# raadyn/aztotmd

Measured on AMD Instinct MI355X. Metric: ns_per_day, higher is better.
Workload: dtype f64; 1 GPU; 1 000 188 Ar, LJ rc 8.5 A, FCC 63^3 a=5.735 jitter 0.15, dt 1 fs, NVE, init_vel zero (BASELINE config '1 000 000 Ar LJ', SURVEY C4); n_atoms=1000188, n_cells=68921, decomposition=single GPU, transport=single GPU, rccl_ranks=0, pair_variant=0, sort_interval=105, sort_violations=0, pair_lists=1, cells_without_list=0, kernel_timing=off

## Files before the change

aztotmd_amd/api.py:

```python
import ctypes as C
import enum
import os
import subprocess

import numpy as np

_HERE = os.path.dirname(os.path.abspath(__file__))
_LIB = None

STAT_FIELDS = ("step", "time", "engTot", "engKin", "engVdW", "engCoul", "engElecField", "engTemp", "engPot", "temperature",
               "posMom", "negMom", "posCross", "negCross", "pressure", "pairs_dropped", "n_cells", "nose_chit", "nose_conint",
               "engBond", "engAngle", "engCoulRec", "engCoulConst", "sort_interval", "sort_violations", "pair_lists", "cells_without_list", "rebuilds", "skin")


class AztotError(RuntimeError):
    def __init__(self, code, msg):
        super().__init__("aztot error %d: %s" % (code, msg))
        self.code = code


class _Species(C.Structure):
    _fields_ = [("name", C.c_char * 8), ("mass_amu", C.c_double), ("charge", C.c_double), ("frozen", C.c_int32),
                ("radA", C.c_double), ("radB", C.c_double), ("mxEng", C.c_double)]


class _Vdw(C.Structure):
    _fields_ = [("spec_a", C.c_int32), ("spec_b", C.c_int32), ("type", C.c_int32), ("rcut", C.c_double), ("p", C.c_double * 5)]


class _Control(C.Structure):
    _fields_ = [("timestep", C.c_double), ("nstep", C.c_int32), ("nequil", C.c_int32), ("eqfreq", C.c_int32),
                ("temperature", C.c_double), ("tstat_type", C.c_int32), ("tstat_tau", C.c_double), ("elec_type", C.c_int32),
                ("r_real", C.c_double), ("alpha", C.c_double), ("init_vel", C.c_int32), ("init_vel_par", C.c_double * 3),
                ("elecfield", C.c_double * 3), ("use_cell_list", C.c_int32), ("cell_list", C.c_double), ("stat", C.c_int32),
                ("ewald_k", C.c_int32 * 3)]


_dp = C.POINTER(C.c_double)
_ip = C.POINTER(C.c_int32)


class _System(C.Structure):
    _fields_ = [("n_atoms", C.c_int32), ("n_species", C.c_int32), ("n_vdw", C.c_int32), ("box", C.c_double * 3),
                ("types", _ip), ("x", _dp), ("y", _dp), ("z", _dp), ("vx", _dp), ("vy", _dp), ("vz", _dp),
                ("species", C.POINTER(_Species)), ("vdw", C.POINTER(_Vdw)), ("control", _Control)]


class _BondType(C.Structure):
    _fields_ = [("spec_a", C.c_int32), ("spec_b", C.c_int32), ("type", C.c_int32), ("p", C.c_double * 5)]


class _AngleType(C.Structure):
    _fields_ = [("central", C.c_int32), ("type", C.c_int32), ("k", C.c_double), ("cos0", C.c_double)]


class _Bonded(C.Structure):
    _fields_ = [("n_bond_types", C.c_int32), ("n_angle_types", C.c_int32), ("n_bonds", C.c_int32), ("n_angles", C.c_int32),
                ("bond_types", C.POINTER(_BondType)), ("angle_types", C.POINTER(_AngleType)),
                ("bond_a", _ip), ("bond_b", _ip), ("bond_type", _ip),
                ("angle_c", _ip), ("angle_l1", _ip), ("angle_l2", _ip), ("angle_type", _ip)]


class _Options(C.Structure):
    _fields_ = [("struct_size", C.c_uint32), ("device", C.c_int32), ("initial_forces", C.c_int32), ("center_box", C.c_int32), ("seed", C.c_uint64),
                ("pair_variant", C.c_int32), ("cell_size", C.c_double), ("use_graph", C.c_int32), ("profile", C.c_int32),
                ("sort_every", C.c_int32), ("skin", C.c_double), ("waves_per_cell", C.c_int32), ("energies_every_step", C.c_int32),
                ("loopback_ranks", C.c_int32), ("reserved", C.c_int32 * 5)]


class _Stats(C.Structure):
    _fields_ = [("step", C.c_int64), ("time", C.c_double), ("engTot", C.c_double), ("engKin", C.c_double), ("engVdW", C.c_double),
                ("engCoul", C.c_double), ("engElecField", C.c_double), ("engTemp", C.c_double), ("engPot", C.c_double),
                ("temperature", C.c_double), ("posMom", C.c_double * 3), ("negMom", C.c_double * 3), ("posCross", C.c_int64 * 3),
                ("negCross", C.c_int64 * 3), ("pressure", C.c_double), ("pairs_dropped", C.c_int64), ("n_cells", C.c_int64),
                ("nose_chit", C.c_double), ("nose_conint", C.c_double), ("engBond", C.c_double), ("engAngle", C.c_double),
                ("engCoulRec", C.c_double), ("engCoulConst", C.c_double), ("sort_interval", C.c_int64), ("sort_violations", C.c_int64),
                ("pair_lists", C.c_int64), ("cells_without_list", C.c_int64), ("rebuilds", C.c_int64), ("skin", C.c_double)]


class _CnColumn(C.Structure):
    _fields_ = [("central", C.c_int32), ("ligand", C.c_int32), ("radius", C.c_double)]


class _AdfColumn(C.Structure):
    _fields_ = [("central", C.c_int32), ("ligand_a", C.c_int32), ("ligand_b", C.c_int32), ("reserved", C.c_int32), ("radius_a", C.c_double), ("radius_b", C.c_double)]


class _BooParams(C.Structure):
    _fields_ = [("radius", C.c_double), ("central_mask", C.c_int32), ("ligand_mask", C.c_int32), ("n_orders", C.c_int32), ("orders", C.c_int32 * 4),
                ("n_bins", C.c_int32), ("reserved", C.c_int32)]


class _Stress(C.Structure):
    _fields_ = [("step", C.c_int64), ("time", C.c_double), ("volume", C.c_double), ("kinetic", C.c_double * 6), ("virial", C.c_double * 6),
                ("pressure", C.c_double * 6), ("pressure_iso", C.c_double), ("eng_vdw", C.c_double), ("eng_coul", C.c_double),
                ("pairs", C.c_int64), ("pairs_dropped", C.c_int64)]


class _Clock(C.Structure):
    _fields_ = [("step", C.c_int64), ("nose_chit", C.c_double), ("nose_conint", C.c_double), ("eng_kin", C.c_double)]


class _State(C.Structure):
    _fields_ = [("n_atoms", C.c_int32)] + [(k, _dp) for k in ("x", "y", "z", "vx", "vy", "vz", "fx", "fy", "fz", "U", "radius")] + [("types", _ip)]


SENDRECV_FN = C.CFUNCTYPE(C.c_int, C.c_void_p, C.c_int, C.c_void_p, C.c_int64, C.c_int, C.c_void_p, C.c_int64, C.POINTER(C.c_int64))
ALLREDUCE_FN = C.CFUNCTYPE(C.c_int, C.c_void_p, _dp, C.c_int)

EXPORTS = ("aztot_device_count", "aztot_device_synchronize", "aztot_init_md", "aztot_model_create", "aztot_model_set_bonded", "aztot_model_query", "aztot_model_species_name", "aztot_model_nucleus_name", "aztot_free_md", "aztot_default_options",
           "aztot_init_device", "aztot_free_device", "aztot_step", "aztot_sync", "aztot_forces", "aztot_get_stats", "aztot_species_crossings", "aztot_md_to_host",
           "aztot_set_state", "aztot_get_clock", "aztot_set_clock", "aztot_cell_table", "aztot_kernel_times", "aztot_reset_kernel_times", "aztot_set_profile", "aztot_comm_id_bytes", "aztot_comm_make_id", "aztot_comm_selftest", "aztot_comm_ranks",
           "aztot_init_device_slab", "aztot_rdf_setup", "aztot_rdf_sample", "aztot_rdf_reset", "aztot_rdf_shape", "aztot_rdf_counts", "aztot_rdf_values",
           "aztot_cn_setup", "aztot_cn_sample", "aztot_cn_shape", "aztot_cn_per_atom", "aztot_cn_table",
           "aztot_tcf_setup", "aztot_tcf_sample", "aztot_tcf_reset", "aztot_tcf_shape", "aztot_tcf_sums", "aztot_tcf_values",
           "aztot_stress_setup", "aztot_stress_sample", "aztot_stress_get", "aztot_stress_per_atom",
           "aztot_adf_setup", "aztot_adf_sample", "aztot_adf_reset", "aztot_adf_shape", "aztot_adf_edges", "aztot_adf_counts", "aztot_adf_values",
           "aztot_adf_neighbours",
           "aztot_sk_setup", "aztot_sk_sample", "aztot_sk_reset", "aztot_sk_shape", "aztot_sk_vectors", "aztot_sk_amplitudes", "aztot_sk_sums", "aztot_sk_values",
           "aztot_boo_setup", "aztot_boo_sample", "aztot_boo_reset", "aztot_boo_shape", "aztot_boo_per_atom", "aztot_boo_qlm", "aztot_boo_counts", "aztot_boo_values",
           "aztot_last_error", "aztot_version")

RDF_KINDS = {"species": 0, "nuclei": 1}
CN_KINDS = {"species": 0, "nuclei": 1}


class DebugBit(enum.IntFlag):
    DBG_BUILD_PHASE_MASK = 3
    DBG_ALWAYS_CLEANUP = 4
    DBG_FOLD_DRIFT = 8
    DBG_NO_FOLD_DRIFT = 16
    DBG_WIDE_ENTRIES = 32
    DBG_HITS_BESIDE_TILE = 64
    DBG_KICK_EVERY_STEP = 128
    DBG_LARGE_KICK_PATH = 256
    DBG_GENERIC_PAIR = 512
    DBG_KEEP_VDW_CUT_TEST = 1024
    DBG_STAGE_ONLY = 2048
    DBG_SLAB_GRAPH = 4096
    DBG_FIXED_INTERVAL = 8192
    DBG_OVERLAP_HALO = 16384
    DBG_NO_LISTS = 32768
    DBG_SHORT_LISTS = 65536
    DBG_NO_FUSE_NEXT = 131072
    DBG_FUSE_NEXT = 262144
    DBG_CHECK_EVERY_ATOM = 524288
    DBG_LIST_STATS = 2097152
    DBG_KICK_POST_SPLIT = 4194304
    DBG_GRAPH_ALWAYS = 8388608
    DBG_PLAIN_ONE_ATOM = 16777216
    DBG_NO_BOUNDARY_RADI = 33554432
    DBG_ONE_WAVE_PER_CELL = 67108864
    DBG_ENERGIES_EVERY_STEP = 134217728
    DBG_SETTLE_EVERY_CALL = 268435456
    DBG_NO_FOLD_KICK = 536870912
    DBG_FOLD_KICK = 1073741824


def library_path():
    return os.environ.get("AZTOT_LIB") or os.path.join(_HERE, "libaztot.so")


def build_library(force=False):
    src_dir = os.path.join(_HERE, "csrc")
    so = library_path()
    newest = max(os.path.getmtime(os.path.join(src_dir, f)) for f in os.listdir(src_dir) if f.endswith((".h", ".hip", ".cpp")) or f == "Makefile")
    hdr = os.path.join(os.path.dirname(_HERE), "include", "aztot.h")
    newest = max(newest, os.path.getmtime(hdr))
    def stale():
        return force or not os.path.exists(so) or os.path.getmtime(so) < newest

    if stale():
        import fcntl
        with open(os.path.join(src_dir, ".build.lock"), "w") as lock:
            fcntl.flock(lock, fcntl.LOCK_EX)
            try:
                if stale():
                    subprocess.check_call(["make", "-C", src_dir, "all"], stdout=subprocess.DEVNULL)
            finally:
                fcntl.flock(lock, fcntl.LOCK_UN)
    return so


def lib():
    global _LIB
    if _LIB is None:
        so = library_path()
        if not os.path.exists(so):
            raise ImportError("aztotmd_amd: %s is missing - build it with `python -c 'import __graft_entry__ as g; g.build()'` "
                              "(hipcc --offload-arch=gfx950). There is no CPU fallback for the hot path." % so)
        L = C.CDLL(so)
        L.aztot_last_error.restype = C.c_char_p
        L.aztot_version.restype = C.c_char_p
        L.aztot_init_md.argtypes = [C.c_char_p, C.POINTER(C.c_void_p)]
        L.aztot_model_create.argtypes = [C.POINTER(_System), C.POINTER(C.c_void_p)]
        L.aztot_model_query.argtypes = [C.c_void_p, C.c_char_p, _dp, C.c_int]
        L.aztot_model_set_bonded.argtypes = [C.c_void_p, C.POINTER(_Bonded)]
        L.aztot_free_md.argtypes = [C.c_void_p]
        L.aztot_free_md.restype = None
        L.aztot_default_options.argtypes = [C.POINTER(_Options)]
        L.aztot_default_options.restype = None
        L.aztot_init_device.argtypes = [C.c_void_p, C.POINTER(_Options), C.POINTER(C.c_void_p)]
        L.aztot_init_device_slab.argtypes = [C.c_void_p, C.POINTER(_Options), C.c_int, C.c_int, C.c_void_p, SENDRECV_FN, ALLREDUCE_FN,
                                             C.c_void_p, C.POINTER(C.c_void_p)]
        L.aztot_free_device.argtypes = [C.c_void_p]
        L.aztot_free_device.restype = None
        L.aztot_step.argtypes = [C.c_void_p, C.c_int]
        L.aztot_sync.argtypes = [C.c_void_p]
        L.aztot_forces.argtypes = [C.c_void_p]
        L.aztot_get_stats.argtypes = [C.c_void_p, C.POINTER(_Stats)]
        L.aztot_species_crossings.argtypes = [C.c_void_p, C.POINTER(C.c_int64), C.c_int]
        L.aztot_md_to_host.argtypes = [C.c_void_p, C.POINTER(_State)]
        L.aztot_set_state.argtypes = [C.c_void_p, C.POINTER(_State)]
        L.aztot_get_clock.argtypes = [C.c_void_p, C.POINTER(_Clock)]
        L.aztot_set_clock.argtypes = [C.c_void_p, C.POINTER(_Clock)]
        L.aztot_cell_table.argtypes = [C.c_void_p, _ip, _ip, C.c_int, _ip, C.c_int]
        L.aztot_kernel_times.argtypes = [C.c_void_p, C.c_char_p, C.c_int, _dp, C.POINTER(C.c_int64), C.c_int]
        L.aztot_reset_kernel_times.argtypes = [C.c_void_p]
        L.aztot_set_profile.argtypes = [C.c_void_p, C.c_int]
        L.aztot_comm_make_id.argtypes = [C.c_void_p]
        L.aztot_comm_selftest.argtypes = [C.c_int]
        L.aztot_comm_ranks.argtypes = [C.c_void_p]
        L.aztot_model_species_name.argtypes = [C.c_void_p, C.c_int, C.c_char_p, C.c_int]
        L.aztot_model_nucleus_name.argtypes = [C.c_void_p, C.c_int, C.c_char_p, C.c_int]
        L.aztot_rdf_setup.argtypes = [C.c_void_p, C.c_double, C.c_double, C.c_int]
        L.aztot_rdf_sample.argtypes = [C.c_void_p]
        L.aztot_rdf_reset.argtypes = [C.c_void_p]
        L.aztot_rdf_shape.argtypes = [C.c_void_p, C.c_int, _ip, _ip]
        L.aztot_rdf_counts.argtypes = [C.c_void_p, C.c_int, C.POINTER(C.c_int64), C.POINTER(C.c_uint64), C.c_int]
        L.aztot_rdf_values.argtypes = [C.c_void_p, C.c_int, _dp, _dp, C.c_int]
        L.aztot_cn_setup.argtypes = [C.c_void_p, C.c_int, C.POINTER(_CnColumn), C.c_int]
        L.aztot_cn_sample.argtypes = [C.c_void_p, C.c_int]
        L.aztot_cn_shape.argtypes = [C.c_void_p, C.c_int, _ip, _ip, _ip]
        L.aztot_cn_per_atom.argtypes = [C.c_void_p, C.c_int, _ip, C.c_int]
        L.aztot_cn_table.argtypes = [C.c_void_p, C.c_int, C.POINTER(C.c_int64), C.c_int]
        L.aztot_tcf_setup.argtypes = [C.c_void_p, C.c_int, C.c_int]
        L.aztot_tcf_sample.argtypes = [C.c_void_p]
        L.aztot_tcf_reset.argtypes = [C.c_void_p]
        L.aztot_tcf_shape.argtypes = [C.c_void_p, _ip, _ip, C.POINTER(C.c_int64)]
        L.aztot_tcf_sums.argtypes = [C.c_void_p, C.c_int, C.c_int, C.POINTER(C.c_int64), _dp, _dp, C.c_int]
        L.aztot_tcf_values.argtypes = [C.c_void_p, C.c_int, C.c_int, _dp, _dp, C.c_int]
        L.aztot_stress_setup.argtypes = [C.c_void_p]
        L.aztot_stress_sample.argtypes = [C.c_void_p]
        L.aztot_stress_get.argtypes = [C.c_void_p, C.POINTER(_Stress)]
        L.aztot_stress_per_atom.argtypes = [C.c_void_p, _dp, C.c_int]
        L.aztot_adf_setup.argtypes = [C.c_void_p, C.c_int, C.POINTER(_AdfColumn), C.c_int]
        L.aztot_adf_sample.argtypes = [C.c_void_p]
        L.aztot_adf_reset.argtypes = [C.c_void_p]
        L.aztot_adf_shape.argtypes = [C.c_void_p, _ip, _ip, C.POINTER(C.c_int64)]
        L.aztot_adf_edges.argtypes = [C.c_void_p, _dp, C.c_int]
        L.aztot_adf_counts.argtypes = [C.c_void_p, C.POINTER(C.c_int64), C.POINTER(C.c_uint64), C.c_int]
        L.aztot_adf_values.argtypes = [C.c_void_p, _dp, _dp, C.c_int]
        L.aztot_adf_neighbours.argtypes = [C.c_void_p, _ip, C.c_int]
        L.aztot_sk_setup.argtypes = [C.c_void_p, C.c_double, C.c_double, C.c_int]
        L.aztot_sk_sample.argtypes = [C.c_void_p]
        L.aztot_sk_reset.argtypes = [C.c_void_p]
        L.aztot_sk_shape.argtypes = [C.c_void_p, _ip, _ip, _ip, C.POINTER(C.c_int64)]
        L.aztot_sk_vectors.argtypes = [C.c_void_p, _ip, _ip, C.c_int]
        L.aztot_sk_amplitudes.argtypes = [C.c_void_p, _dp, C.c_int]
        L.aztot_sk_sums.argtypes = [C.c_void_p, C.POINTER(C.c_int64), _dp, C.c_int]
        L.aztot_sk_values.argtypes = [C.c_void_p, _dp, _ip, _dp, _dp, C.c_int]
        L.aztot_boo_setup.argtypes = [C.c_void_p, C.POINTER(_BooParams)]
        L.aztot_boo_sample.argtypes = [C.c_void_p]
        L.aztot_boo_reset.argtypes = [C.c_void_p]
        L.aztot_boo_shape.argtypes = [C.c_void_p, _ip, _ip, _ip, _ip, C.POINTER(C.c_int64)]
        L.aztot_boo_per_atom.argtypes = [C.c_void_p, _ip, _dp, C.c_int]
        L.aztot_boo_qlm.argtypes = [C.c_void_p, _dp, C.c_int]
        L.aztot_boo_counts.argtypes = [C.c_void_p, C.POINTER(C.c_int64), C.POINTER(C.c_uint64), _dp, C.POINTER(C.c_uint64), C.c_int]
        L.aztot_boo_values.argtypes = [C.c_void_p, _dp, _dp, _dp, C.c_int]
        _LIB = L
    return _LIB


def _check(rc):
    if rc < 0:
        raise AztotError(rc, lib().aztot_last_error().decode("utf-8", "replace"))
    return rc


def _f8(a):
    return np.ascontiguousarray(a, dtype=np.float64)


class Model:

    def __init__(self, handle, keep=None):
        self.h = handle
        self._keep = keep

    @classmethod
    def from_dir(cls, directory):
        h = C.c_void_p()
        _check(lib().aztot_init_md(os.fsencode(directory), C.byref(h)))
        return cls(h)

    @classmethod
    def from_case(cls, case):
        N = len(case["types"])
        types = np.ascontiguousarray(case["types"], dtype=np.int32)
# ... 519 lines not shown
```

aztotmd_amd/csrc/device_md.h:

```cpp
#pragma once
#include <cstdint>

namespace aztot {

constexpr int kSpecCap = 16;

struct AtomArrays
{
    double *x, *y, *z;
    double *vx, *vy, *vz;
    double *fx, *fy, *fz;
    double *U, *rad;
    int32_t *type;
    int32_t *id;
};

struct RefPos { double *x, *y, *z; };

struct SpecTable
{
    double mass[kSpecCap], charge[kSpecCap], rMhdt[kSpecCap];
    double radA[kSpecCap], radB[kSpecCap], mxEng[kSpecCap];
    int32_t charged[kSpecCap], frozen[kSpecCap];
};

struct DevPot
{
    int32_t type, use_radii;
    double p0, p1, p2, p3, p4, r2cut;
};

struct DevBondType { int32_t type, pad; double p0, p1, p2, p3, p4; };
struct DevAngleType { double k, cos0; };
struct BondEntry { int32_t partner; int32_t typeFirst; };
struct AngleEntry { int32_t roleType, c, l1, l2; };
struct BondedTables
{
    const int32_t* bondStart;
    const BondEntry* bondEnt;
    const int32_t* angStart;
    const AngleEntry* angEnt;
    const DevBondType* btypes;
    const DevAngleType* atypes;
    int32_t* idxOfId;
};

enum { EWK_NEW_L = 1, EWK_NEW_LM = 2 };
struct EwaldK
{
    int32_t l, m, n, flags;
    double rkx, rky, rkz, akk;
};
struct EwaldW
{
    int32_t l, m, n;
    int32_t kPlus, kMinus;
};
struct EwaldG
{
    int32_t l, m, nLo, nHi, kStart;
};
struct EwaldTables
{
    const EwaldK* kv;
    const EwaldW* work;
    const EwaldG* groups;
    double* T;
    int32_t nK, nW, nG, kx, ky, kz, nBlocksA;
    double* partial;
    double* S;
    double scale, scale2;
};

struct SplitArgs
{
    int n = 1;
    double *fx = nullptr, *fy = nullptr, *fz = nullptr;
    int32_t* arrived = nullptr;
    int capacity = 0;
};

enum DebugBit : unsigned
{
    DBG_BUILD_PHASE_MASK = 3,
    DBG_ALWAYS_CLEANUP = 4,
    DBG_FOLD_DRIFT = 8,
    DBG_NO_FOLD_DRIFT = 16,
    DBG_WIDE_ENTRIES = 32,
    DBG_HITS_BESIDE_TILE = 64,
    DBG_KICK_EVERY_STEP = 128,
    DBG_LARGE_KICK_PATH = 256,
    DBG_GENERIC_PAIR = 512,
    DBG_KEEP_VDW_CUT_TEST = 1024,
    DBG_STAGE_ONLY = 2048,
    DBG_SLAB_GRAPH = 4096,
    DBG_FIXED_INTERVAL = 8192,
    DBG_OVERLAP_HALO = 16384,
    DBG_NO_LISTS = 32768,
    DBG_SHORT_LISTS = 65536,
    DBG_NO_FUSE_NEXT = 131072,
    DBG_FUSE_NEXT = 262144,
    DBG_CHECK_EVERY_ATOM = 524288,
    DBG_LIST_STATS = 2097152,
    DBG_KICK_POST_SPLIT = 4194304,
    DBG_GRAPH_ALWAYS = 8388608,
    DBG_PLAIN_ONE_ATOM = 16777216,
    DBG_NO_BOUNDARY_RADI = 33554432,
    DBG_ONE_WAVE_PER_CELL = 67108864,
    DBG_ENERGIES_EVERY_STEP = 134217728,
    DBG_SETTLE_EVERY_CALL = 268435456,
    DBG_NO_FOLD_KICK = 536870912,
    DBG_FOLD_KICK = 1073741824
};

enum KickFuse
{
    KICK_NONE = 0,
    KICK_SECOND = 1,
    KICK_BOTH = 2,
    KICK_DRIFT = 3
};

enum PotSet { POTSET_GENERIC = 0, POTSET_ONE_FAMILY = 2, POTSET_ONE_SURK = 4 };

struct StepParams
{
    int32_t nOwned;
    int32_t nTotal;
    int32_t nSpec;
    int32_t single_lj;
    double L[3], invL[3], half[3];
    double dt;
    int32_t nc[3];
    int32_t ncxLocal, cx0;
    int32_t nCellLocal;
    int32_t hw[3];
    int32_t nOff[3];
    double csz[3], icsz[3];
    double r2Max;
    int32_t elec_type, use_radii;
    double alpha, el_scale, el_scale2, daipi2, rReal, fcoul, sqrtpi;
    double E[3];
    int32_t tstat, nEq, freqEq, debugMask;
    double tKin, revDegFree, rkB;
    double rQmass, qMassTau2;
    double revLight, radFrac, radThr, numPi;
    uint64_t seed;
    int32_t nAtGlobal, potSet;
    double xlo, xhi;
    int32_t rank, nranks;
    int32_t fuseKick;
    int32_t vdwFamily;
    int32_t cycleStep;
    int32_t boundSkip;
    double lazySlack2;
    double pruneR2;
    double ljDropR2;
    int32_t optimistic, pad3;
};

enum PartialSlot
{
    PS_EFIELD = 0, PS_MOM_XN, PS_MOM_XP, PS_MOM_YN, PS_MOM_YP, PS_MOM_ZN, PS_MOM_ZP,
    PS_CNT_XN, PS_CNT_XP, PS_CNT_YN, PS_CNT_YP, PS_CNT_ZN, PS_CNT_ZP,
    PS_EVDW, PS_ECOUL, PS_DROPPED, PS_EKIN, PS_ETEMP, PS_EBOND, PS_EANGLE, PS_COUNT
};

struct DevStats
{
    long long step;
    long long stepAtSort;
    double engKin, engVdW, engCoul, engElecField, engTemp, engTot, engPot, temperature;
    double engBond, engAngle;
    double engCoulRec, engCoulConst;
    double mom[6];
    long long cross[6];
    long long dropped;
    double vscale;
    double vscaleBegin;
    double ekSim;
    double chit, conint;
    long long pendingKick;
    double local[PS_COUNT];
    unsigned long long specCross[kSpecCap * 6];
};

struct RdfGrid
{
    int nc[3];
    int nCell;
    int halfShell;
    double L[3], invL[3], half[3], icsz[3];
    double r2max, idr;
    int nBins;
    int nSpec, nPairS;
    int nNucl, nPairN;
    int nucl[kSpecCap];
};

constexpr int kCnLive = 15;
struct CnParams
{
    int shift;
    int inclusive;
    int countSelf;
    int maxLive;
    int nCols;
};

}
```

aztotmd_amd/csrc/engine.h:

```cpp
#pragma once
#include <hip/hip_runtime.h>

#include <algorithm>
#include <memory>
#include <stdexcept>
#include <string>
#include <vector>

#include "device_md.h"
#include "device_resources.h"
#include "list_store.h"
#include "model.h"
#include "msg_layout.h"
#include "samplers.h"

namespace aztot {

struct Counts;
struct PairLists; struct PairLaunch;

struct ArgError : std::runtime_error
{
    using std::runtime_error::runtime_error;
};
// ... 13 lines not shown
    void forces(bool withBonded = true);
    void get_stats(aztot_stats& out);
    void species_crossings(int64_t* out, int cap);
    void md_to_host(aztot_state& out);
    void set_state(const aztot_state& in);
    void get_clock(aztot_clock& out);
    void set_clock(const aztot_clock& in);
    int cell_table(int32_t dims[3], int32_t* cellStart, int capCells, int32_t* atomId, int capAtoms);
    int kernel_times(std::vector<KernelTimer>& out);
    void reset_kernel_times();
    void set_profile(bool on) { sync_all(); profile_ = on; }
    int n_atoms_global() const { return model_.nAt; }
    int comm_ranks() const { return xch_ ? xch_->comm_ranks() : 0; }
    void sync_all();
    Samplers& samplers() { return *samplers_; }

private:
    void step_body(int nsteps);
    bool settle_now() const;
    void settle();
    void mark_failed(const char* what) noexcept;
    bool unsettled_ = false;
    std::string failed_;
    void construct();
    void release();
    void check_launch(const char* where);
    void choose_cells();
    void allocate();
    void alloc_atoms(AtomArrays& A, bool zero);
    void upload_initial();
    void upload_bonded();
    void upload_ewald();
    void launch_ewald();
    void sort_and_forces(int stepMode, bool withBonded = true);
    void launch_step_kernels();
    void run_steps(int nsteps);
    void launch_pair();
    int pair_variant() const;
    void exchange_halo();
    void collect_and_finalize(unsigned slotMask);
    void finish_steps();
    void check_overflow();
    void sync();
    DevStats read_stats();
    Counts read_counts();
    template <typename F> void timed(const char* name, F&& launch) { if (!profile_ || capturing_) launch(); else timers_.timed(name, stream_, launch); }
    template <typename T> T* dev_alloc(size_t n, bool zero = false) { return mem_.alloc<T>(n, zero, stream_); }
    PairLaunch pair_launch(const StepParams& Q);
    AtomArrays& cur() { return buf_[cur_]; }
    AtomArrays& oth() { return buf_[cur_ ^ 1]; }
    int left() const { return (rank_ + nranks_ - 1) % nranks_; }
    int right() const { return (rank_ + 1) % nranks_; }
    void quiesce() override { sync_all(); }
    AtomArrays begin_sample() override;
    void end_sample(const char* where) override { check_launch(where); sync(); }
    void launch_timed(const char* name, const std::function<void()>& launch) override { timed(name, launch); }
    Samplers::PairTables pair_tables() override { return {P_, S_, dPots_, hostStep_}; }

    Model model_;
    aztot_options opt_;
    unsigned debug_ = 0;
    StepParams P_{};
    SpecTable S_{};
    int rank_, nranks_;
    Exchanger* xch_;
    std::unique_ptr<Exchanger> ownedXch_;

    hipStream_t stream_ = nullptr;
    hipStream_t commStream_ = nullptr;
    hipEvent_t evIntegrated_ = nullptr, evHalo_ = nullptr;
    DeviceArena mem_;
    bool profile_ = false;
    KernelTimers timers_;
    int capacity_ = 0;
    int maxBlocks_ = 0;
    AtomArrays buf_[2]{};
    int cur_ = 0;
    DevPot* dPots_ = nullptr;
    int32_t *dCellOf_ = nullptr, *dSlotOf_ = nullptr, *dCellCount_ = nullptr, *dCellStart_ = nullptr;
    int32_t* dChunkTot_ = nullptr;
    int32_t *dTmpId_ = nullptr, *dTmpSrc_ = nullptr, *dTmpCell_ = nullptr, *dCellOfSorted_ = nullptr;
    double* dPartials_ = nullptr;
    DevStats* dStats_ = nullptr;
    Counts* dCounts_ = nullptr;
    double *dPhotons_ = nullptr, *dUvx_ = nullptr, *dUvy_ = nullptr, *dUvz_ = nullptr;
    double* dStage_ = nullptr;
    double* dEkGlobal_ = nullptr;
    char* dMsg_[4] = {nullptr, nullptr, nullptr, nullptr};
    MsgLayout lay_{};
    SplitArgs split_{};
    BondedTables bonded_{};
    bool hasBonded_ = false;
    EwaldTables ew_{};
    bool hasEwald_ = false;
    bool thermoTouched_ = false;

    ListStore lists_;
    bool listsValid_ = false;
    PinnedReadback hUnlisted_;
    int unlistedState_ = 0;
    bool unlistedAtLook_ = false;

    static constexpr int kNoSort = 1 << 30;
    bool lazyOn_ = false;
    int lazyK_ = 1;
    int lazyCap_ = 32;
    long long lazyViolations_ = 0;
    int lazyWindow_ = 8;
    int sinceLook_ = 0;
    double lazyMargin_ = 1.15;
    bool lazyMeasured_ = false;
    double lastLookLen_ = 0.0;
    int sinceSort_ = kNoSort;
    long long rebuilds_ = 0;
    double lazySlack_ = 0.0;
    double skinTarget_ = 0.0;
    RefPos ref_{};
    bool carryAgreed_ = false;
    void forget_interval() { sinceSort_ = kNoSort; listsValid_ = false; carryAgreed_ = false; }
    void void_measurement() { lazyMeasured_ = false; lazyWindow_ = 8; sinceLook_ = 0; }
    void set_interval(int K) { if (K != lazyK_) { lazyK_ = K; drop_graphs(); } }
    void clear_violation_flag();
    int window_cap() const { return nranks_ > 1 ? 64 : 256; }
    void look_sync();
    PinnedReadback hLook_;
    bool adapt_sort_interval();
    void look(bool callEnd);
    void prepare_next_call();
    int halo_[5] = {0, 0, 0, 0, 0};
    PinnedReadback hHalo_;
    int32_t* dHaloInfo_ = nullptr;
    bool haloInfoPending_ = false;
    void take_halo_info();
    void post_count_exchange();
    void adopt_halo_info(const int32_t* h);

    long long hostStep_ = 0;
    bool equil_phase() const { return P_.nEq > 0 && hostStep_ < P_.nEq; }

    double lastMom_[6] = {0, 0, 0, 0, 0, 0};
    double pressure_ = 0.0;
    long long lastPresStep_ = 0;

    std::unique_ptr<Samplers> samplers_;

    struct BufState { int cur; double* xyz[2][3]; double* alt[2][3]; };
    struct LaunchNotes
    {
        int pairBlocksUsed = 0;
        int blocksEver = 0;
        bool ekinFromPair = false;
        bool lastStepEquil = false;
    } notes_;
    struct GraphSlot { BufState before, after; LaunchNotes notes; hipGraph_t graph = nullptr; hipGraphExec_t exec = nullptr; int entryBytes = 2; };
    void adopt_launch_notes(const LaunchNotes& n) { const int ever = std::max(notes_.blocksEver, n.blocksEver); notes_ = n; notes_.blocksEver = ever; }
    std::vector<GraphSlot> graphs_;
    int graphCycle_ = 0;
    bool capturing_ = false;
    void drop_graphs();
    BufState buf_state() const;
    GraphSlot* graph_for_state(int cycle);
    int graph_cycle() const;
    bool can_graph() const;
    void set_buf_state(const BufState& b);

    bool lazyKick_ = false;
    bool kickOwed_ = false;
    bool fuseEpilogue_ = false;
    bool fuseNow_ = false;
    bool foldKickOk_ = false;
    bool foldKick_ = false;
    bool kickFolded_ = false;
    bool foldDriftOk_ = false;
    bool overlapHalo_ = false;
    int candMode_ = 0;
    double* altXyz_[2][3] = {{nullptr, nullptr, nullptr}, {nullptr, nullptr, nullptr}};
    bool fuseNextOk_ = false;
    bool fuseNext_ = false;
    bool fuseNextTstat_ = false;
    bool pairClosedStep_ = false;
    bool preIntegrated_ = false;
    int stepsLeftInRun_ = 0;

    struct DynState
    {
        AtomArrays A{};
        void *stats = nullptr, *counts = nullptr;
        double* partials = nullptr;
    };
    struct Snapshot : DynState
    {
        BufState buf{};
        long long hostStep = 0;
        bool valid = false;
    } snap_;
    long long stepsSinceSnap_ = 0;
    DynState live() { return DynState{cur(), dStats_, dCounts_, dPartials_}; }
    void copy_state(DynState from, DynState to);
    bool optimistic_ = false;
    int safeLooks_ = 1;
    int rollbacks_ = 0;
    void choose_optimism();
    bool rollback_on() const { return lazyOn_ && (nranks_ > 1 || optimistic_); }
    void take_snapshot();
    void replay_from_snapshot();
};

}
```

aztotmd_amd/csrc/engine.hip:

```cpp
#include "engine.h"

#include <algorithm>
#include <cmath>
#include <array>
#include <cstring>
#include <cstddef>
#include <cstdio>
#include <cstdlib>
#include <stdexcept>
#include <tuple>

#include "exchange.h"
#include "bonded.hip.h"
#include "ewald.hip.h"
#include "kernels.hip.h"
#include "pair_tile.hip.h"
#include "pair_list.hip.h"
#include "rdf.hip.h"
#include "cn.hip.h"
#include "adf.hip.h"
#include "sk.hip.h"
#include "tcf.hip.h"
#include "slab.hip.h"

// ... 303 lines not shown
    {
        buf_[k].x = b.xyz[k][0]; buf_[k].y = b.xyz[k][1]; buf_[k].z = b.xyz[k][2];
        for (int d = 0; d < 3; d++) altXyz_[k][d] = b.alt[k][d];
    }
}

void Engine::release()
{
    if (stream_) (void)hipStreamSynchronize(stream_);
    drop_graphs();
    if (evIntegrated_) (void)hipEventDestroy(evIntegrated_);
    if (evHalo_) (void)hipEventDestroy(evHalo_);
    evIntegrated_ = evHalo_ = nullptr;
    if (commStream_) { (void)hipStreamSynchronize(commStream_); (void)hipStreamDestroy(commStream_); }
    commStream_ = nullptr;
    if (stream_) (void)hipStreamDestroy(stream_);
    stream_ = nullptr;
}

void Engine::check_launch(const char* where)
{
    if (capturing_) return;
    check_hip(hipGetLastError(), where);
}

static std::array<double**, 11> double_arrays(AtomArrays& A) { return {&A.x, &A.y, &A.z, &A.vx, &A.vy, &A.vz, &A.fx, &A.fy, &A.fz, &A.U, &A.rad}; }

void Engine::alloc_atoms(AtomArrays& A, bool zero)
{
    for (double** pp : double_arrays(A)) *pp = dev_alloc<double>((size_t)capacity_, zero);
    A.type = dev_alloc<int32_t>((size_t)capacity_, zero); A.id = dev_alloc<int32_t>((size_t)capacity_, zero);
}

void Engine::allocate()
{
    const int N = model_.nAt;
    if (nranks_ > 1)
    {
        const int ncx = P_.nc[0], hw = P_.hw[0];
        std::vector<long long> hist(ncx, 0);
        for (int i = 0; i < N; i++)
        {
            int gx = (int)std::floor(model_.x[i] * P_.icsz[0]);
            gx %= ncx; if (gx < 0) gx += ncx;
            hist[gx]++;
        }
        long long maxLayer = 0, maxRun = 0, window = 0;
        for (int g = 0; g < ncx; g++)
        {
            maxLayer = std::max(maxLayer, hist[g]);
            long long run = 0;
            for (int k = 0; k < hw; k++) run += hist[(g + k) % ncx];
            maxRun = std::max(maxRun, run);
        }
        for (int l = 0; l < P_.ncxLocal; l++) window += hist[(((P_.cx0 + l) % ncx) + ncx) % ncx];
        capacity_ = (int)(std::ceil((window + maxRun) * 1.25) + 4096);
        lay_.haloCap = (int)std::min<double>((double)N, std::ceil(maxRun * 1.25) + 1024);
        lay_.migCap = (int)std::min<double>((double)N, std::ceil(maxLayer * 0.03) + 1024);
    }
    else capacity_ = N;
    {
        const int cells = pair_tile_cells(P_);
        int n = 1;
        if (pair_tile_supported(P_) && !(debug_ & DBG_ONE_WAVE_PER_CELL))
            while (n < 8 && cells * n * 2 <= 4096 && n * 2 <= P_.nOff[0] * P_.nOff[1]) n *= 2;
        if (n == 1 && pair_tile_supported(P_) && !(debug_ & DBG_ONE_WAVE_PER_CELL))
        {
            const double vol = swept_volume(P_.csz[0], P_.csz[1], P_.csz[2], model_.rMax);
            const double density = (double)model_.nAt / (model_.L[0] * model_.L[1] * model_.L[2]);
            if (density * vol > 1.15 * kTileCap && P_.nOff[0] * P_.nOff[1] >= 2) n = 2;
        }
        if (opt_.waves_per_cell == 1 || opt_.waves_per_cell == 2 || opt_.waves_per_cell == 4 || opt_.waves_per_cell == 8) n = opt_.waves_per_cell;
        split_.n = n;
        split_.capacity = capacity_;
    }
    const int pairBlocks = std::max(div_up(capacity_, kBlock), pair_tile_grid(P_) * std::max(split_.n, kListMaxWaves) + 24 + 3 * pair_cleanup_grid(pair_tile_cells(P_)));
    maxBlocks_ = std::max(div_up(capacity_, kBlock), pairBlocks) + 1;
    const size_t nAtoms = (size_t)capacity_, nCells = (size_t)(P_.nCellLocal + 1);
    for (AtomArrays& A : buf_) alloc_atoms(A, true);
    dCellOf_ = dev_alloc<int32_t>(nAtoms); dSlotOf_ = dev_alloc<int32_t>(nAtoms);
    dTmpId_ = dev_alloc<int32_t>(nAtoms); dTmpSrc_ = dev_alloc<int32_t>(nAtoms); dTmpCell_ = dev_alloc<int32_t>(nAtoms); dCellOfSorted_ = dev_alloc<int32_t>(nAtoms);
    dCellCount_ = dev_alloc<int32_t>(nCells, true); dCellStart_ = dev_alloc<int32_t>(nCells, true);
    dPartials_ = dev_alloc<double>((size_t)PS_COUNT * maxBlocks_, true); dStats_ = dev_alloc<DevStats>(1);
    {
        DevStats zero;
        std::memset(&zero, 0, sizeof(zero));
        zero.vscale = 1.0;
        zero.vscaleBegin = 1.0;
        HIP_CHECK(hipMemcpy(dStats_, &zero, sizeof(DevStats), hipMemcpyHostToDevice));
    }
    if (split_.n > 1)
    {
        const size_t nb = (size_t)split_.n * capacity_;
        split_.fx = dev_alloc<double>(nb); split_.fy = dev_alloc<double>(nb); split_.fz = dev_alloc<double>(nb);
        split_.arrived = dev_alloc<int32_t>((size_t)P_.nCellLocal, true);
    }
    dCounts_ = dev_alloc<Counts>(1); dChunkTot_ = dev_alloc<int32_t>((size_t)(div_up(P_.nCellLocal, kScanChunk) + 1));
    dEkGlobal_ = dev_alloc<double>(2); dStage_ = dev_alloc<double>((size_t)PS_COUNT * kCollectParts, true);
    if (nranks_ > 1)
    {
        for (int k = 0; k < 4; k++) dMsg_[k] = dev_alloc<char>(lay_.bytes(), true);
        dHaloInfo_ = dev_alloc<int32_t>(HI_COUNT, true);
    }
    const int ns = model_.nSpec();
    std::vector<DevPot> pots((size_t)ns * ns);
    for (int a = 0; a < ns; a++)
        for (int b = 0; b < ns; b++)
        {
            const PairPot& p = model_.pot(a, b);
            DevPot& d = pots[(size_t)a * ns + b];
            d.type = p.type; d.use_radii = p.use_radii; d.p0 = p.p0; d.p1 = p.p1; d.p2 = p.p2; d.p3 = p.p3; d.p4 = p.p4; d.r2cut = p.r2cut;
            if (p.type == AZTOT_VDW_LJ) { const double s6 = p.p1 * p.p1 * p.p1; d.p3 = p.p2 * s6; d.p4 = 2.0 * p.p2 * s6 * s6; }
        }
    {
        const Model& m = model_;
        double slack = 1e300;
        bool widenOk = true;
        for (int k = 0; k < 3; k++)
        {
            slack = std::min(slack, 0.49 * (P_.hw[k] * P_.csz[k] - m.rMax));
            if (P_.nc[k] < 2 * (P_.hw[k] + 1) + 1) widenOk = false;
        }
        const int sortEvery = opt_.sort_every;
        lazyOn_ = sortEvery != 1 && (widenOk || nranks_ > 1) && m.rMax > 0 && slack > 1e-3 && m.E[0] == 0.0 && m.E[1] == 0.0 &&
                  m.E[2] == 0.0 && pair_tile_supported(P_);
        lazyCap_ = sortEvery > 1 ? std::min(sortEvery, kLazyCapMax) : kLazyCapMax;
        if (lazyOn_ && (debug_ & DBG_FIXED_INTERVAL)) lazyK_ = lazyCap_;
        slack = std::min(slack, skinTarget_ > 0.0 ? 0.5 * 1.25 * skinTarget_ : 0.012 * m.rMax);
        lazySlack_ = lazyOn_ ? slack : 0.0;
        P_.lazySlack2 = lazySlack_ * lazySlack_;
        const double rp = m.rMax + 2.0 * lazySlack_;
        P_.pruneR2 = rp * rp * (1.0 + 1e-12);
        if (lazyOn_)
        {
            ref_.x = dev_alloc<double>(nAtoms); ref_.y = dev_alloc<double>(nAtoms); ref_.z = dev_alloc<double>(nAtoms);
            if (capacity_ < (1 << 26) && !(debug_ & DBG_NO_LISTS))
                lists_.create(P_, m, opt_, capacity_, rp, stream_, rank_);
        }
    }
    dPots_ = dev_alloc<DevPot>(pots.size());
    HIP_CHECK(hipMemcpyAsync(dPots_, pots.data(), sizeof(DevPot) * pots.size(), hipMemcpyHostToDevice, stream_));
    HIP_CHECK(hipStreamSynchronize(stream_));
}

int ListStore::waves_wanted(double tileRecords, int iters) const
{
    const double tileBytes = tileRecords * (P_->single_lj ? 24.0 : (pair_list_tab_mode(*P_) ? 25.0 : 32.0));
    if (tileBytes > 26.0 * 1024 || iters > 192) return 4;
    return (tileBytes > 13.0 * 1024 || iters > 96) ? 2 : 1;
}

void ListStore::create(const StepParams& P, const Model& m, const aztot_options& opt, int capacity, double listRadius, hipStream_t stream, int rank)
{
    P_ = &P; stream_ = stream; capacity_ = capacity; rank_ = rank;
    forcedWaves_ = (opt.waves_per_cell == 1 || opt.waves_per_cell == 2 || opt.waves_per_cell == 4) ? opt.waves_per_cell : 0;
    if (P.ncxLocal > 1023 || P.nc[1] > 1023 || P.nc[2] > 1023) throw std::runtime_error("more than 1023 cells along an axis");
    int devLds = 0;
    HIP_CHECK(hipDeviceGetAttribute(&devLds, hipDeviceAttributeMaxSharedMemoryPerBlock, opt.device));
    ldsMax_ = (size_t)std::max(devLds, 64 * 1024);
    const double a = P.csz[0], b = P.csz[1], c = P.csz[2], r = listRadius;
    const double vol = swept_volume(a, b, c, r);
    const double density = (double)m.nAt / (m.L[0] * m.L[1] * m.L[2]);
    const double perCell = density * a * b * c, partners = density * 4.18879020478639 * r * r * r;
    waves = forcedWaves_ ? forcedWaves_ : waves_wanted(density * vol, 0);
    int cand = (int)(density * vol * 1.5) + 64;
    int iters = (int)(partners * 1.25 / list_slices(list_atoms_per_wave(std::min(kWave * waves, (int)(1.6 * perCell) + 6), waves))) + 4;
    cand = std::max(kListMinCand * waves, (cand + 63) & ~63);
    iters = std::max(2 * kListMinIter, (iters + 7) & ~7);
    if (const char* e = std::getenv("AZTOT_CAND_CAP")) cand = std::atoi(e);
    if (const char* e = std::getenv("AZTOT_ITER_CAP")) iters = std::atoi(e);
    try { allocate(cand, iters); }
    catch (const std::exception&)
    {
        (void)hipGetLastError();
        release();
    }
}

void ListStore::allocate(int candCapNew, int iterCapNew)
{
    release();
    const StepParams& P = *P_;
    candCapNew = std::max(kListMinCand * waves, std::min((candCapNew + 63) & ~63, kListCandMax));
    iterCapNew = std::max(kListMinIter, std::min((iterCapNew + 7) & ~7, kListIterMax));
    PairLists probe;
    probe.candCap = probe.candLds = probe.stageLds = candCapNew; probe.iterCap = probe.iterLds = iterCapNew; probe.recBytes = pair_list_rec_bytes(P); probe.waves = waves;
    probe.buildGroups = (P.debugMask & DBG_HITS_BESIDE_TILE) ? 0 : 1;
    while (candCapNew > kListMinCand && (pair_list_lds_bytes(P, probe) > ldsMax_ || build_lists_lds_bytes(probe) > ldsMax_))
    {
        candCapNew -= 64;
        probe.candCap = probe.candLds = probe.stageLds = candCapNew;
    }
    while (iterCapNew > 2 * kListMinIter && build_lists_lds_bytes(probe) > ldsMax_) { iterCapNew -= 8; probe.iterCap = probe.iterLds = iterCapNew; }
    const size_t nc = (size_t)P.nCellLocal;
    cand = mem_.alloc<uint32_t>(nc * candCapNew, true, stream_);
    meta = mem_.alloc<int32_t>(4 * nc, false, stream_);
    pairs = mem_.alloc<uint16_t>(nc * (size_t)waves * (size_t)iterCapNew * kWave, true, stream_);
    report = mem_.alloc<int32_t>(LR_COUNT, true, stream_); rel = mem_.alloc<float4>((size_t)capacity_ + kWave, true, stream_);
    candCap = candCapNew; iterCap = iterCapNew;
    candLds = stageLds = candCapNew; iterLds = iterCapNew;
    buildGroups = groups_that_fit(4 * waves, stageLds, iterLds);
    entryBytes = entryNext = 2;
    {
        std::vector<int32_t> mx(4 * nc, 0);
        const int ncy = P.nc[1], ncz = P.nc[2];
        for (size_t c = 0; c < nc; c++)
        {
            const int cz = (int)(c % ncz), cy = (int)((c / ncz) % ncy), lx = (int)(c / ((size_t)ncy * ncz));
            mx[4 * c] = -1; mx[4 * c + 1] = lx | (cy << 10) | (cz << 20);
        }
        HIP_CHECK(hipMemcpyAsync(meta, mx.data(), sizeof(int32_t) * 4 * nc, hipMemcpyHostToDevice, stream_));
        HIP_CHECK(hipStreamSynchronize(stream_));
    }
    on = true;
    if (std::getenv("AZTOT_VERBOSE"))
        std::fprintf(stderr, "aztot: pair lists for %zu cells: %d candidates, %d iterations per cell (%.1f MB), LDS %zu B (list kernel) / %zu B (builder)\n", nc, candCap, iterCap,
                     (double)(nc * ((size_t)candCap * 4 + (size_t)iterCap * 128)) / 1e6, pair_list_lds_bytes(P, pair_lists()), build_lists_lds_bytes(pair_lists()));
}

void ListStore::regrow(int candCapNew, int iterCapNew)
{
    try { allocate(candCapNew, iterCapNew); }
    catch (const std::exception& e)
    {
        (void)hipGetLastError();
        release();
        if (std::getenv("AZTOT_VERBOSE")) std::fprintf(stderr, "aztot: rank %d: no room for larger pair lists (%s): the run goes on without lists\n", rank_, e.what());
    }
}

void ListStore::release() noexcept
{
    if (stream_) (void)hipStreamSynchronize(stream_);
    mem_.release();
    cand = nullptr; meta = nullptr; pairs = nullptr; report = nullptr; rel = nullptr;
    on = false;
}

PairLists ListStore::pair_lists() const
{
    PairLists pl;
    if (on)
    {
        pl.cand = cand; pl.meta = meta; pl.pairs = pairs; pl.noList = report;
        pl.candCap = candCap; pl.iterCap = iterCap; pl.candLds = candLds; pl.stageLds = stageLds; pl.iterLds = iterLds; pl.recBytes = pair_list_rec_bytes(*P_); pl.waves = waves;
        pl.buildGroups = buildGroups;
        pl.entryBytes = entryBytes; pl.entryScale = entryBytes == 1 ? 1 : pair_list_entry_scale(*P_);
        pl.rel = rel;
    }
    return pl;
}

int ListStore::tile_records_for(int maxT) const
{
    constexpr size_t kLdsBlock = 1280;
    PairLists L = pair_lists();
    const bool roomy = P_->nranks == 1 && capacity_ <= 2 * kFuseKickMaxAtoms;
    int need = std::max(4 * kWave, std::min(candCap, roomy ? maxT + maxT / 16 + 4 : maxT + maxT / 100 + 1));
    if (maxT <= 255 && P_->nranks == 1 && waves == 1) need = 4 * kWave;
    if (need <= 4 * kWave) return need;
    L.candLds = need;
    const size_t blocks = (pair_list_lds_bytes(*P_, L) + kLdsBlock - 1) / kLdsBlock;
    int best = need;
    for (int c = need + 1; c <= candCap; c++)
    {
        L.candLds = c;
        if ((pair_list_lds_bytes(*P_, L) + kLdsBlock - 1) / kLdsBlock > blocks) break;
        best = c;
    }
    return best;
}

int ListStore::stage_records_for(int maxStaged) const
{
    return std::max(4 * kWave, std::min(candCap, (maxStaged + maxStaged / 16 + 4 + 127) & ~127));
}

int ListStore::groups_that_fit(int want, int stageLdsNew, int iterLdsNew) const
{
    if (P_->debugMask & DBG_HITS_BESIDE_TILE) return 0;
    constexpr size_t kLdsBlock = 1280;
    PairLists L;
    L.stageLds = stageLdsNew; L.iterLds = iterLdsNew; L.waves = waves;
    L.buildGroups = std::max(1, std::min(want, 4 * waves));
    while (L.buildGroups > 1 && build_lists_lds_bytes(L) > ldsMax_) L.buildGroups--;
    const size_t blocks = (build_lists_lds_bytes(L) + kLdsBlock - 1) / kLdsBlock;
    while (L.buildGroups < 4 * waves)
    {
        L.buildGroups++;
        if ((build_lists_lds_bytes(L) + kLdsBlock - 1) / kLdsBlock > blocks || build_lists_lds_bytes(L) > ldsMax_) { L.buildGroups--; break; }
    }
    return L.buildGroups;
}

void ListStore::lds_for(const int32_t* rep, int& candLdsNew, int& stageLdsNew, int& iterLdsNew, int& groupsNew) const
{
    candLdsNew = tile_records_for(rep[LR_MAX_TILE]);
    stageLdsNew = stage_records_for(rep[LR_MAX_STAGED]);
    iterLdsNew = std::max(2 * kListMinIter, std::min(iterCap, (rep[LR_MAX_ITERS] + rep[LR_MAX_ITERS] / 8 + 2 + 7) & ~7));
    if (entryNext == 1 && ((iterLdsNew + 15) & ~15) <= iterCap) iterLdsNew = (iterLdsNew + 15) & ~15;
    groupsNew = groups_that_fit((rep[LR_MAX_ATOMS] + 15) / 16, stageLdsNew, iterLdsNew);
}

bool ListStore::narrow_fits(int maxTile, int candLdsNew, int wavesNew) const
{
    return P_->nranks == 1 && !(P_->debugMask & DBG_WIDE_ENTRIES) && !wideForGood_ && wavesNew == 1 && list_preload(candLdsNew) == 4 && maxTile <= 255;
}

bool ListStore::tighten(const int32_t* rep, bool* formatChanged)
{
    if (formatChanged) *formatChanged = false;
    if (rep[LR_TILE_FULL] != 0 || rep[LR_LIST_FULL] != 0 || rep[LR_KEPT_FULL] != 0 || rep[LR_MASK_FULL] != 0 || rep[LR_MAX_STAGED] <= 0) return false;
    int c, s, i, g;
    lds_for(rep, c, s, i, g);
    bool changed = false;
    if (entryNext == 2 && narrow_fits(rep[LR_MAX_TILE], std::min(candLds, c), waves))
    {
        entryNext = 1;
        lds_for(rep, c, s, i, g);
        changed = true;
        if (formatChanged) *formatChanged = true;
    }
    if (c >= candLds && s >= stageLds && i >= iterLds && g >= buildGroups) return changed;
    candLds = std::min(candLds, c); stageLds = std::min(stageLds, s); iterLds = std::min(iterLds, i); buildGroups = std::min(buildGroups, g);
    if (std::getenv("AZTOT_VERBOSE"))
        std::fprintf(stderr, "aztot: list LDS sized from the first recording: tile %d, staging %d, %d iterations, %d mask groups: %zu B (list kernel) / %zu B (builder)\n", candLds, stageLds, iterLds,
                     buildGroups, pair_list_lds_bytes(*P_, pair_lists()), build_lists_lds_bytes(pair_lists()));
    return true;
}

ListStore::Verdict ListStore::adapt(const int32_t* rep, unsigned debug)
{
    Verdict v;
    const bool frozen = debug & DBG_SHORT_LISTS;
    if (debug & DBG_LIST_STATS)
    {
        std::fprintf(stderr, "aztot: per cell: %.2f list iterations, %.1f candidates staged, %.1f kept, %.2f atoms; %.1f %% of the cells walk more than 16 iterations (%d-byte entries)\n",
                     (double)rep[LR_SUM_ITERS] / rep[LR_RECORDED], (double)rep[LR_SUM_STAGED] / rep[LR_RECORDED], (double)rep[LR_SUM_CANDS] / rep[LR_RECORDED],
                     (double)rep[LR_SUM_ATOMS] / rep[LR_RECORDED], 100.0 * (double)rep[LR_OVER_16] / rep[LR_RECORDED], entryBytes);
        HIP_CHECK(hipMemset(&report[LR_SUM_ITERS], 0, sizeof(int32_t) * 4));
        HIP_CHECK(hipMemset(&report[LR_OVER_16], 0, sizeof(int32_t)));
    }
    HIP_CHECK(hipMemsetAsync(&report[LR_UNLISTED], 0, sizeof(int32_t) * 2, stream_));
    HIP_CHECK(hipMemsetAsync(&report[LR_TILE_FULL], 0, sizeof(int32_t) * 3, stream_));
    HIP_CHECK(hipMemsetAsync(&report[LR_MASK_FULL], 0, sizeof(int32_t), stream_));
    const int tileFull = rep[LR_TILE_FULL], keptFull = rep[LR_KEPT_FULL], listFull = rep[LR_LIST_FULL], maskFull = rep[LR_MASK_FULL], recorded = rep[LR_RECORDED], unlisted = rep[LR_UNLISTED];
    if (std::getenv("AZTOT_VERBOSE"))
        std::fprintf(stderr, "aztot: lists recorded since the last look: %d cells, %d of them without a list (%d: staging full, %d: tile full, %d: list full, %d: mask buffer full); most staged %d of %d (LDS %d), largest tile %d (LDS %d), longest list %d of %d (LDS %d), most atoms %d (LDS %d groups, builder %zu B)\n",
                     recorded, unlisted, tileFull, keptFull, listFull, maskFull, rep[LR_MAX_STAGED], candCap, stageLds, rep[LR_MAX_TILE], candLds, rep[LR_MAX_ITERS], iterCap, iterLds, rep[LR_MAX_ATOMS], buildGroups,
                     build_lists_lds_bytes(pair_lists()));
    int candLdsNew, stageLdsNew, iterLdsNew, groupsNew;
    lds_for(rep, candLdsNew, stageLdsNew, iterLdsNew, groupsNew);
    if (tileFull > 0) stageLdsNew = std::min(candCap, std::max(stageLdsNew, stageLds + 128));
    if (keptFull > 0) candLdsNew = std::min(candCap, std::max(candLdsNew, candLds + 32));
    if (listFull > 0) iterLdsNew = std::min(iterCap, std::max(iterLdsNew, iterLds + 8));
    groupsNew = groups_that_fit((rep[LR_MAX_ATOMS] + 15) / 16, stageLdsNew, iterLdsNew);
    if (frozen) { candLdsNew = candLds; stageLdsNew = stageLds; iterLdsNew = iterLds; groupsNew = buildGroups; }
    const int wWant = std::max(waves, waves_wanted((double)rep[LR_MAX_TILE], rep[LR_MAX_ITERS]));
    const int wavesNew = (wWant > waves && !forcedWaves_ && !frozen) ? wWant : waves;
    if (entryNext == 1 && (rep[LR_MAX_TILE] > 255 || keptFull > 0 || !narrow_fits(rep[LR_MAX_TILE], candLdsNew, wavesNew)))
    {
        entryNext = 2; wideForGood_ = true;
        v.rebuild = v.launchChanged = true;
    }
    else if (entryNext == 2 && !frozen && tileFull + keptFull + listFull + maskFull == 0 && narrow_fits(rep[LR_MAX_TILE], candLdsNew, wavesNew))
    {
        entryNext = 1;
        v.launchChanged = true;
        lds_for(rep, candLdsNew, stageLdsNew, iterLdsNew, groupsNew);
    }
    if (wWant > waves && !forcedWaves_ && !frozen)
    {
        const int itersNew = std::max(2 * kListMinIter, ((int)(rep[LR_MAX_ITERS] * (double)waves / wWant * 1.3) + 8 + 7) & ~7);
        const int candNew = std::max(candCap, kListMinCand * wWant);
        waves = wWant;
        regrow(candNew, itersNew);
        v.rebuild = v.launchChanged = true;
        return v;
    }
    const bool capFull = (tileFull > 0 && stageLds == candCap) || (keptFull > 0 && candLds == candCap) || (listFull > 0 && iterLds == iterCap);
    if (capFull && !frozen && (double)(tileFull + keptFull + listFull) > ((P_->nranks == 1 && growths < 3) ? 0.0 : 0.0005 * (double)recorded))
    {
        const int candNew = tileFull + keptFull > 0 ? std::min(kListCandMax, (candCap * 3 / 2 + 63) & ~63) : candCap;
        const int itersNew = listFull > 0 ? std::min(kListIterMax, (iterCap * 2 + 7) & ~7) : iterCap;
        v.launchChanged = true;
        if (growths < 3 && (candNew > candCap || itersNew > iterCap)) { growths++; regrow(candNew, itersNew); v.rebuild = true; }
    }
    else if (candLdsNew != candLds || stageLdsNew != stageLds || iterLdsNew != iterLds || groupsNew != buildGroups)
    {
        candLds = candLdsNew; stageLds = stageLdsNew; iterLds = iterLdsNew; buildGroups = groupsNew;
        v.launchChanged = true;
    }
    if (on && (double)unlisted > 0.02 * (double)recorded && !frozen && tileFull + keptFull + listFull + maskFull < unlisted / 2)
    {
        on = false;
        v.launchChanged = true;
    }
    return v;
}

void Engine::upload_bonded()
{
    const Model& m = model_;
    const size_t nb = m.bondA.size(), na = m.angC.size();
    hasBonded_ = (nb + na) > 0;
    if (!hasBonded_) return;
    const int N = m.nAt;
    auto up = [&](const void* src, size_t bytes) {
        void* p = dev_alloc<char>(bytes);
        if (bytes) HIP_CHECK(hipMemcpy(p, src, bytes, hipMemcpyHostToDevice));
        return p;
    };
    std::vector<int32_t> bs(N + 1, 0), as(N + 1, 0);
    for (size_t k = 0; k < nb; k++) { bs[m.bondA[k] + 1]++; bs[m.bondB[k] + 1]++; }
    for (size_t k = 0; k < na; k++) { as[m.angC[k] + 1]++; as[m.angL1[k] + 1]++; as[m.angL2[k] + 1]++; }
    for (int i = 0; i < N; i++) { bs[i + 1] += bs[i]; as[i + 1] += as[i]; }
    std::vector<BondEntry> be(2 * nb);
    std::vector<AngleEntry> ae(3 * na);
    {
        std::vector<int32_t> fill(bs.begin(), bs.end() - 1);
        for (size_t k = 0; k < nb; k++)
        {
            be[fill[m.bondA[k]]++] = BondEntry{m.bondB[k], m.bondT[k] | (1 << 30)};
            be[fill[m.bondB[k]]++] = BondEntry{m.bondA[k], m.bondT[k]};
        }
        fill.assign(as.begin(), as.end() - 1);
        for (size_t k = 0; k < na; k++)
        {
            const int32_t c = m.angC[k], l1 = m.angL1[k], l2 = m.angL2[k], t = m.angT[k] << 2;
            ae[fill[c]++] = AngleEntry{t | 0, c, l1, l2};
            ae[fill[l1]++] = AngleEntry{t | 1, c, l1, l2};
            ae[fill[l2]++] = AngleEntry{t | 2, c, l1, l2};
        }
    }
    std::vector<DevBondType> bt(m.bondTypes.size() + 1);
    std::memset(bt.data(), 0, sizeof(DevBondType) * bt.size());
    for (size_t k = 0; k < m.bondTypes.size(); k++)
    {
        const BondType& b = m.bondTypes[k];
        bt[k + 1] = DevBondType{b.type, 0, b.p[0], b.p[1], b.p[2], b.p[3], b.p[4]};
    }
    std::vector<DevAngleType> at(m.angleTypes.size() + 1, DevAngleType{0.0, 0.0});
    for (size_t k = 0; k < m.angleTypes.size(); k++) at[k + 1] = DevAngleType{m.angleTypes[k].k, m.angleTypes[k].cos0};
    bonded_.bondStart = (const int32_t*)up(bs.data(), sizeof(int32_t) * bs.size());
    bonded_.bondEnt = (const BondEntry*)up(be.data(), sizeof(BondEntry) * be.size());
    bonded_.angStart = (const int32_t*)up(as.data(), sizeof(int32_t) * as.size());
    bonded_.angEnt = (const AngleEntry*)up(ae.data(), sizeof(AngleEntry) * ae.size());
    bonded_.btypes = (const DevBondType*)up(bt.data(), sizeof(DevBondType) * bt.size());
    bonded_.atypes = (const DevAngleType*)up(at.data(), sizeof(DevAngleType) * at.size());
    std::vector<int32_t> none(N, -1);
    bonded_.idxOfId = (int32_t*)up(none.data(), sizeof(int32_t) * (size_t)N);
}

void Engine::upload_ewald()
{
    const Model& m = model_;
    hasEwald_ = m.elec_type == AZTOT_ELEC_EWALD && !m.kvecs.empty();
    if (!hasEwald_) return;
    std::vector<EwaldK> kv(m.kvecs.size());
    for (size_t k = 0; k < kv.size(); k++)
    {
        const KVec& a = m.kvecs[k];
        int flags = 0;
        if (k == 0 || m.kvecs[k - 1].l != a.l) flags |= EWK_NEW_L | EWK_NEW_LM;
        else if (m.kvecs[k - 1].m != a.m) flags |= EWK_NEW_LM;
        kv[k] = EwaldK{a.l, a.m, a.n, flags, a.rkx, a.rky, a.rkz, a.akk};
    }
    EwaldK* dkv = dev_alloc<EwaldK>(kv.size());
    HIP_CHECK(hipMemcpy(dkv, kv.data(), sizeof(EwaldK) * kv.size(), hipMemcpyHostToDevice));
    ew_.kv = dkv;
    std::map<std::tuple<int, int, int>, int> slot;
    std::vector<EwaldW> work;
    for (size_t k = 0; k < kv.size(); k++)
    {
        const auto key = std::make_tuple(kv[k].l, kv[k].m, std::abs(kv[k].n));
        auto it = slot.find(key);
        if (it == slot.end()) { slot[key] = (int)work.size(); work.push_back(EwaldW{kv[k].l, kv[k].m, std::abs(kv[k].n), -1, -1}); it = slot.find(key); }
        if (kv[k].n >= 0) work[it->second].kPlus = (int)k; else work[it->second].kMinus = (int)k;
    }
    EwaldW* dw = dev_alloc<EwaldW>(work.size());
    HIP_CHECK(hipMemcpy(dw, work.data(), sizeof(EwaldW) * work.size(), hipMemcpyHostToDevice));
    ew_.work = dw; ew_.nW = (int)work.size();
    std::vector<EwaldG> groups;
    for (size_t k = 0; k < kv.size(); k++)
    {
        if (!groups.empty() && groups.back().l == kv[k].l && groups.back().m == kv[k].m && groups.back().nHi + 1 == kv[k].n) groups.back().nHi = kv[k].n;
        else groups.push_back(EwaldG{kv[k].l, kv[k].m, kv[k].n, kv[k].n, (int)k});
    }
    EwaldG* dg = dev_alloc<EwaldG>(groups.size());
    HIP_CHECK(hipMemcpy(dg, groups.data(), sizeof(EwaldG) * groups.size(), hipMemcpyHostToDevice));
    ew_.groups = dg; ew_.nG = (int)groups.size();
    ew_.T = dev_alloc<double>(2 * kv.size());
    ew_.nK = (int)kv.size(); ew_.kx = m.ewald_k[0]; ew_.ky = m.ewald_k[1]; ew_.kz = m.ewald_k[2];
    ew_.nBlocksA = std::max(1, std::min(1024, div_up(capacity_, kEwTile)));
    ew_.partial = dev_alloc<double>(2 * (size_t)ew_.nK * ew_.nBlocksA);
    ew_.S = dev_alloc<double>(2 * (size_t)ew_.nK);
    HIP_CHECK(hipMemset(ew_.S, 0, sizeof(double) * 2 * (size_t)ew_.nK));
    ew_.scale = m.el_scale; ew_.scale2 = m.el_scale2;
    {
        const size_t ldsTab = sizeof(double) * 2 * (size_t)kEwTile * (ew_.kx + ew_.ky + ew_.kz);
        const size_t ldsForce = ldsTab + sizeof(double) * 3 * kEwTile * kEwSlices;
        int devMax = 0;
        HIP_CHECK(hipDeviceGetAttribute(&devMax, hipDeviceAttributeMaxSharedMemoryPerBlock, opt_.device));
        const size_t hwMax = std::max<size_t>((size_t)devMax, 160 * 1024);
        if (ldsForce > hwMax)
            throw std::runtime_error("elec pme: kx + ky + kz = " + std::to_string(ew_.kx + ew_.ky + ew_.kz) + " harmonics need " + std::to_string(ldsForce) +
                                     " B of LDS per workgroup, more than the " + std::to_string(hwMax) + " B a CU has (use fewer k-vectors or elec fenn)");
        if (ldsTab > 64 * 1024) HIP_CHECK(hipFuncSetAttribute((const void*)k_ewald_sfac, hipFuncAttributeMaxDynamicSharedMemorySize, (int)ldsTab));
        if (ldsForce > 64 * 1024) HIP_CHECK(hipFuncSetAttribute((const void*)k_ewald_force, hipFuncAttributeMaxDynamicSharedMemorySize, (int)ldsForce));
    }
    DevStats s;
    HIP_CHECK(hipMemcpy(&s, dStats_, sizeof(DevStats), hipMemcpyDeviceToHost));
    s.engCoulConst = m.engElec1;
    HIP_CHECK(hipMemcpy(dStats_, &s, sizeof(DevStats), hipMemcpyHostToDevice));
}

void Engine::launch_ewald()
{
    const size_t lds = sizeof(double) * 2 * (size_t)kEwTile * (ew_.kx + ew_.ky + ew_.kz);
    timed("ewald_sfac", [&] {
        hipLaunchKernelGGL(k_ewald_sfac, dim3(ew_.nBlocksA), dim3(256), lds, stream_, P_, S_, cur(), dCounts_, ew_);
        hipLaunchKernelGGL(k_ewald_reduce, dim3(div_up(ew_.nK, 64)), dim3(64 * kEwRedGroups), 0, stream_, ew_);
    });
    if (nranks_ > 1) timed("ewald_allreduce", [&] { xch_->allreduce_device(ew_.S, 2 * ew_.nK, stream_); });
    timed("ewald_energy", [&] { hipLaunchKernelGGL(k_ewald_energy, dim3(1), dim3(256), 0, stream_, ew_, dStats_); });
    timed("ewald_force", [&] {
        hipLaunchKernelGGL(k_ewald_force, dim3(div_up(capacity_, kEwTile)), dim3(kEwTile * kEwSlices), lds + sizeof(double) * 3 * kEwTile * kEwSlices,
                           stream_, P_, S_, cur(), dCounts_, ew_);
    });
    check_launch("Ewald kernels");
}

void Engine::upload_initial()
{
    const Model& m = model_;
    const int N = m.nAt;
    std::vector<int32_t> ids; ids.reserve(capacity_);
    for (int i = 0; i < N; i++)
    {
        if (nranks_ > 1)
        {
            int gx = (int)std::floor(m.x[i] * P_.icsz[0]);
            gx %= P_.nc[0]; if (gx < 0) gx += P_.nc[0];
            const int lo = P_.cx0 + P_.hw[0], hi = lo + P_.ncxLocal - 2 * P_.hw[0];
            if (gx < lo || gx >= hi) continue;
        }
        ids.push_back(i);
    }
    const int n = (int)ids.size();
    if (n > capacity_) throw std::runtime_error("slab capacity exceeded at initialisation");
    AtomArrays& A = cur();
    std::vector<double> tmp(std::max(n, 1));
    auto up = [&](double* dst, const std::vector<double>& src) {
        for (int k = 0; k < n; k++) tmp[k] = src[ids[k]];
        HIP_CHECK(hipMemcpy(dst, tmp.data(), sizeof(double) * (size_t)n, hipMemcpyHostToDevice));
    };
    up(A.x, m.x); up(A.y, m.y); up(A.z, m.z); up(A.vx, m.vx); up(A.vy, m.vy); up(A.vz, m.vz);
    std::vector<int32_t> ty(std::max(n, 1));
    for (int k = 0; k < n; k++) ty[k] = m.types[ids[k]];
    HIP_CHECK(hipMemcpy(A.type, ty.data(), sizeof(int32_t) * (size_t)n, hipMemcpyHostToDevice));
    HIP_CHECK(hipMemcpy(A.id, ids.data(), sizeof(int32_t) * (size_t)n, hipMemcpyHostToDevice));
    if (m.tstat_type == AZTOT_TSTAT_RADI)
    {
        std::vector<double> ph(N), ux(kNumUnitVectors), uy(kNumUnitVectors), uz(kNumUnitVectors);
        photon_engs(N, ph.data(), m.Temp, opt_.seed);
        unit_vectors(ux.data(), uy.data(), uz.data());
        auto alloc_up = [&](double*& d, const std::vector<double>& h) {
            d = dev_alloc<double>(h.size());
            HIP_CHECK(hipMemcpy(d, h.data(), sizeof(double) * h.size(), hipMemcpyHostToDevice));
        };
        alloc_up(dPhotons_, ph); alloc_up(dUvx_, ux); alloc_up(dUvy_, uy); alloc_up(dUvz_, uz);
    }
    if (m.tstat_type == AZTOT_TSTAT_RADI || P_.use_radii)
    {
        for (int k = 0; k < n; k++) tmp[k] = initial_radius(opt_.seed, (uint64_t)ids[k]);
        HIP_CHECK(hipMemcpy(A.rad, tmp.data(), sizeof(double) * (size_t)n, hipMemcpyHostToDevice));
    }
    Counts c{};
    c.ownedBegin = 0; c.ownedEnd = n; c.nTotal = n; c.srcBegin = 0; c.srcEnd = n;
    HIP_CHECK(hipMemcpy(dCounts_, &c, sizeof(Counts), hipMemcpyHostToDevice));
    if (opt_.initial_forces) forces(false);
}

int Engine::pair_variant() const
{
    int variant = opt_.pair_variant;
    if (variant == 0) variant = pair_tile_supported(P_) ? 2 : 1;
    if (variant == 2 && !pair_tile_supported(P_)) variant = 1;
    return variant;
}

PairLaunch Engine::pair_launch(const StepParams& Q) { return PairLaunch{Q, S_, dPots_, cur(), dCounts_, dCellStart_, dPartials_, maxBlocks_, stream_}; }

void Engine::launch_pair()
{
    const int variant = pair_variant();
    int splitBlocks = 0;
    if (variant == 2)
    {
        StepParams Q = P_;
        Q.fuseKick = fuseNow_ ? KICK_SECOND : KICK_NONE;
        const PairLaunch C = pair_launch(Q);
        const bool wantEnergies = stepsLeftInRun_ == 0 || (debug_ & DBG_ENERGIES_EVERY_STEP);
        if (candMode_ == 1 && lists_.on && !overlapHalo_) lists_.begin_recording();
        const PairLists pl = lists_.pair_lists();
        if (overlapHalo_)
        {
            const int plane = P_.nc[1] * P_.nc[2], hw = P_.hw[0];
            PairRange in, lo, hi;
            in.first = 2 * hw * plane; in.n = (P_.ncxLocal - 4 * hw) * plane;
            lo.first = hw * plane; lo.n = hw * plane;
            hi.first = (P_.ncxLocal - 2 * hw) * plane; hi.n = hw * plane;
            const bool lists = candMode_ == 2 && pl.cand;
            int nb = 0;
            auto run = [&](PairRange& r) {
                r.blockBase = nb;
                if (lists)
                {
                    nb += launch_pair_list(C, r, pl, NextStep(), wantEnergies);
                    nb += launch_pair_cleanup(C, r, pl);
                }
                else
                {
                    launch_pair_tile(C, r, PairLists(), 0, NextStep(), split_);
                    nb += pair_range_grid(r.n) * split_.n;
                }
            };
            timed(lists ? "pair_list" : "pair_tile", [&] {
                run(in);
                HIP_CHECK(hipStreamWaitEvent(stream_, evHalo_, 0));
                run(lo);
                run(hi);
            });
            splitBlocks = nb;
            overlapHalo_ = false;
        }
        else
        {
            if (candMode_ != 0 && pl.cand)
            {
                if (candMode_ == 1)
                {
                    timed("build_lists", [&] { launch_build_lists(C, PairRange(), pl); });
                    listsValid_ = true;
                    unlistedState_ = 0;
                    if (nranks_ > 1 && !capturing_)
                    {
                        hUnlisted_.post(&pl.noList[LR_UNLISTED_NOW], sizeof(int32_t), stream_);
                        hUnlisted_.mark(stream_);
                    }
                }
                else if (nranks_ > 1 && unlistedState_ == 0 && !capturing_ && hUnlisted_.landed())
                    unlistedState_ = (*hUnlisted_.as<int32_t>() == 0) ? 1 : 2;
                const bool skipCleanup = (nranks_ > 1 && unlistedState_ == 1 && candMode_ == 2 && !capturing_) || optimistic_;
                NextStep nx;
                nx.st = dStats_; nx.cnt = dCounts_; nx.R0 = ref_;
                if (fuseNext_) { nx.xn = altXyz_[cur_][0]; nx.yn = altXyz_[cur_][1]; nx.zn = altXyz_[cur_][2]; }
                if (fuseNext_ && fuseNextTstat_) { nx.photons = dPhotons_; nx.uvx = dUvx_; nx.uvy = dUvy_; nx.uvz = dUvz_; pairClosedStep_ = true; }
                else nx.pendingAfter = lazyKick_ ? 1 : -1;
                const bool fold = foldKick_ && skipCleanup && !fuseNext_ && !wantEnergies;
                foldKick_ = false;
                StepParams QL = Q;
                const bool foldDrift = fold && foldDriftOk_;
                if (fold) { QL.fuseKick = foldDrift ? KICK_DRIFT : KICK_BOTH; nx.pendingAfter = 0; kickFolded_ = !foldDrift; }
                if (foldDrift)
                {
                    nx.xd = altXyz_[cur_][0]; nx.yd = altXyz_[cur_][1]; nx.zd = altXyz_[cur_][2];
                    nx.driftBlocks = div_up(div_up(capacity_, 2), kBlock);
                    if (profile_ && !capturing_) timers_.count("fold_drift");
                }
                const PairLaunch CL = pair_launch(QL);
                if (profile_ && !capturing_ && pl.entryBytes == 1) timers_.count("narrow_lists");
                timed("pair_list", [&] { splitBlocks = launch_pair_list(CL, PairRange(), pl, nx, wantEnergies); });
                if (!skipCleanup)
                    timed("pair_cleanup", [&] { splitBlocks += launch_pair_cleanup(C, PairRange(), pl, nx); });
                if (fuseNext_ || foldDrift)
                {
                    AtomArrays& A = cur();
                    std::swap(A.x, altXyz_[cur_][0]); std::swap(A.y, altXyz_[cur_][1]); std::swap(A.z, altXyz_[cur_][2]);
                    preIntegrated_ = true;
                }
            }
            else
                timed("pair_tile", [&] { launch_pair_tile(C, PairRange(), pl, 0, NextStep(), split_); });
        }
    }
    else
        timed("pair_atom", [&] {
            hipLaunchKernelGGL(k_pair_atom, dim3(div_up(capacity_, kBlock)), dim3(kBlock), 0, stream_, P_, S_, dPots_, cur(), dCounts_, dCellStart_,
                               dCellOfSorted_, dPartials_, maxBlocks_);
        });
    if (variant < 2) fuseNow_ = false;
    foldKick_ = false;
    notes_.pairBlocksUsed = (variant == 2) ? (splitBlocks ? splitBlocks : pair_tile_grid(P_) * split_.n) : div_up(capacity_, kBlock);
    notes_.blocksEver = std::max(notes_.blocksEver, std::max(notes_.pairBlocksUsed, div_up(capacity_, kBlock)) + 1);
}

void Engine::take_halo_info()
{
    if (!haloInfoPending_) return;
    hHalo_.wait();
    haloInfoPending_ = false;
    adopt_halo_info(hHalo_.as<int32_t>());
}

void Engine::post_count_exchange()
{
    int32_t* h = dHaloInfo_;
    xch_->exchange_counts(left(), right(), &h[HI_SEND_LEFT], &h[HI_SEND_RIGHT], &h[HI_LEFT_SENDS], &h[HI_RIGHT_SENDS], 2, stream_);
}

void Engine::adopt_halo_info(const int32_t* h)
{
    halo_[0] = h[HI_OWNED_BEGIN]; halo_[1] = h[HI_LEFT_END]; halo_[2] = h[HI_RIGHT_BEGIN]; halo_[3] = h[HI_OWNED_END]; halo_[4] = h[HI_NTOTAL];
    const int ghostsLeft = h[HI_OWNED_BEGIN], ghostsRight = h[HI_NTOTAL] - h[HI_OWNED_END], sendLeft = h[HI_SEND_LEFT], sendRight = h[HI_SEND_RIGHT];
    if (h[HI_RIGHT_SENDS] != ghostsRight || h[HI_RIGHT_HOLDS] != sendRight || h[HI_LEFT_SENDS] != ghostsLeft || h[HI_LEFT_HOLDS] != sendLeft)
        throw std::runtime_error("slab decomposition: the neighbours disagree about their boundary atoms (left boundary: this rank sends " + std::to_string(sendLeft) +
                                 " and holds " + std::to_string(ghostsLeft) + " ghosts, the neighbour holds " + std::to_string(h[HI_LEFT_HOLDS]) + " and sends " + std::to_string(h[HI_LEFT_SENDS]) +
                                 "; right boundary: sends " + std::to_string(sendRight) + ", holds " + std::to_string(ghostsRight) + ", the neighbour holds " +
                                 std::to_string(h[HI_RIGHT_HOLDS]) + " and sends " + std::to_string(h[HI_RIGHT_SENDS]) + "): no coordinate exchange was posted");
}

void Engine::exchange_halo()
{
    timed("exchange", [&] { xch_->exchange(left(), right(), dMsg_[0], dMsg_[1], dMsg_[2], dMsg_[3], lay_.bytes(), stream_); });
    const int recvCap = 2 * (lay_.migCap + lay_.haloCap);
    timed("unpack_halo", [&] {
        hipLaunchKernelGGL(k_unpack, dim3(div_up(recvCap, kBlock)), dim3(kBlock), 0, stream_, P_, cur(), dCounts_, capacity_, lay_, dMsg_[2], dMsg_[3],
                           dCellOf_, dSlotOf_, dCellCount_, dMsg_[0], dMsg_[1]);
    });
}

void Engine::sort_and_forces(int stepMode, bool withBonded)
{
    const int gridAtoms = div_up(capacity_, kBlock);
    const bool integrate_first = stepMode != STEP_BIN_ONLY;
    P_.cycleStep = (stepMode == STEP_PLAIN) ? sinceSort_ + 1 : 0;
    if (stepMode == STEP_PLAIN)
    {
        if (preIntegrated_) preIntegrated_ = false;
        else if (kickFolded_)
        {
            kickFolded_ = false;
            timed("drift", [&] {
                hipLaunchKernelGGL(k_drift_plain2, dim3(div_up(div_up(capacity_, 2), kBlock)), dim3(kBlock), 0, stream_, P_, S_, cur(), dCounts_, dPartials_,
                                   maxBlocks_, dStats_, ref_);
            });
        }
        else if (nranks_ == 1 && P_.tstat != AZTOT_TSTAT_NOSE && !(debug_ & DBG_PLAIN_ONE_ATOM))
            timed("integrate1", [&] {
                hipLaunchKernelGGL(k_integrate_plain2, dim3(div_up(div_up(capacity_, 2), kBlock)), dim3(kBlock), 0, stream_, P_, S_, cur(), dCounts_, dPartials_,
                                   maxBlocks_, dStats_, ref_);
            });
        else
        timed("integrate1", [&] {
            hipLaunchKernelGGL(k_integrate1_bin<STEP_PLAIN>, dim3(gridAtoms), dim3(kBlock), 0, stream_, P_, S_, cur(), dCounts_, dCellOf_, dSlotOf_,
                               dCellCount_, dPartials_, maxBlocks_, lay_, dMsg_[0], dMsg_[1], dStats_, ref_);
        });
        if (nranks_ > 1)
        {
            take_halo_info();
            AtomArrays& A = cur();
            double* arr[4] = {A.x, A.y, A.z, A.rad};
            const int interiorLayers = P_.ncxLocal - 4 * P_.hw[0];
            overlapHalo_ = !profile_ && xch_->device_side() && pair_variant() == 2 && interiorLayers >= 1 && (debug_ & DBG_OVERLAP_HALO);
            if (overlapHalo_)
            {
                HIP_CHECK(hipEventRecord(evIntegrated_, stream_));
                HIP_CHECK(hipStreamWaitEvent(commStream_, evIntegrated_, 0));
            }
            hipStream_t xs = overlapHalo_ ? commStream_ : stream_;
            timed("exchange_coords", [&] {
                xch_->exchange_ranges(left(), right(), arr, P_.use_radii ? 4 : 3, halo_[0], halo_[1] - halo_[0], halo_[2], halo_[3] - halo_[2], 0, halo_[0], halo_[3],
                                      halo_[4] - halo_[3], xs);
            });
            if (overlapHalo_) HIP_CHECK(hipEventRecord(evHalo_, commStream_));
        }
        sinceSort_++;
        candMode_ = 2;
    }
    else
    {
    if (kickFolded_) throw std::runtime_error("a step that needs the forces follows a pair kernel that stored none");
    candMode_ = (stepMode == STEP_RESORT && lazyOn_ && lazyK_ > 1) ? 1 : 0;
    if (integrate_first)
        timed("integrate1_bin", [&] {
            hipLaunchKernelGGL(k_integrate1_bin<STEP_RESORT>, dim3(gridAtoms), dim3(kBlock), 0, stream_, P_, S_, cur(), dCounts_, dCellOf_, dSlotOf_,
                               dCellCount_, dPartials_, maxBlocks_, lay_, dMsg_[0], dMsg_[1], dStats_, ref_);
        });
    else
    {
        HIP_CHECK(hipMemsetAsync(dCellCount_, 0, sizeof(int32_t) * (size_t)(P_.nCellLocal + 1), stream_));
        timed("bin", [&] {
            hipLaunchKernelGGL(k_integrate1_bin<STEP_BIN_ONLY>, dim3(gridAtoms), dim3(kBlock), 0, stream_, P_, S_, cur(), dCounts_, dCellOf_, dSlotOf_,
                               dCellCount_, dPartials_, maxBlocks_, lay_, dMsg_[0], dMsg_[1], dStats_, ref_);
        });
    }
    if (nranks_ > 1) exchange_halo();
    const int nChunks = div_up(P_.nCellLocal, kScanChunk);
    const int setPending = (integrate_first && lazyKick_) ? 1 : 0;
    timed("scan_cells", [&] {
        if (P_.nCellLocal <= kScanSingleMax)
            hipLaunchKernelGGL(k_scan_single, dim3(1), dim3(1024), 0, stream_, P_.nCellLocal, dCellCount_, dCellStart_, dCounts_, dStats_, setPending);
        else
        {
            hipLaunchKernelGGL(k_scan_totals, dim3(nChunks), dim3(kBlock), 0, stream_, P_.nCellLocal, dCellCount_, dChunkTot_);
            hipLaunchKernelGGL(k_scan_apply, dim3(nChunks), dim3(kBlock), 0, stream_, P_.nCellLocal, dCellCount_, dChunkTot_, dCellStart_, dCounts_, dStats_, setPending);
        }
    });
    timed("place", [&] {
        hipLaunchKernelGGL(k_place, dim3(gridAtoms), dim3(kBlock), 0, stream_, dCounts_, dCellOf_, dSlotOf_, dCellStart_, cur().id, dTmpId_, dTmpSrc_,
                           dTmpCell_);
    });
    timed("rank_gather", [&] {
        hipLaunchKernelGGL(k_rank_gather, dim3(gridAtoms), dim3(kBlock), 0, stream_, dCounts_, dCellStart_, dTmpId_, dTmpSrc_, dTmpCell_, cur(), oth(),
                           dCellOfSorted_, (P_.tstat == AZTOT_TSTAT_RADI || P_.use_radii || thermoTouched_) ? 2 : 0, P_, dCounts_, bonded_.idxOfId, ref_,
                           dHaloInfo_, (lists_.on && stepMode == STEP_RESORT && lazyOn_ && lazyK_ > 1) ? &lists_.report[LR_UNLISTED_NOW] : nullptr, lists_.on ? lists_.rel : nullptr);
    });
    cur_ ^= 1;
    sinceSort_ = 0;
    if (!capturing_ && stepMode == STEP_RESORT) rebuilds_++;
    listsValid_ = false;
    if (nranks_ > 1 && lazyOn_ && lazyK_ > 1)
    {
        post_count_exchange();
// ... 168 lines not shown
    stepsSinceSnap_ = 0;
}

void Engine::replay_from_snapshot()
{
    if (!snap_.valid) throw std::runtime_error("lazy re-sort on slab ranks: an atom left its cell's slack and there is no snapshot to go back to");
    sync();
    drop_graphs();
    set_buf_state(snap_.buf);
    copy_state(snap_, live());
    forget_interval(); preIntegrated_ = false; kickFolded_ = false; haloInfoPending_ = false; unlistedState_ = 0;
    kickOwed_ = false;
    hostStep_ = snap_.hostStep;
    if (nranks_ > 1) lazyK_ = 1;
    else
    {
        optimistic_ = false; P_.optimistic = 0;
        rollbacks_ = std::min(rollbacks_ + 1, 12);
        safeLooks_ = 4 << rollbacks_;
    }
    const long long n = stepsSinceSnap_;
    if (std::getenv("AZTOT_VERBOSE")) std::fprintf(stderr, "aztot: rank %d: a skin violation (or a cell without a list) found at a look - %lld steps run again, %s\n", rank_, n, nranks_ > 1 ? "cells rebuilt every step" : "with the clean-up launch");
    if (n > 0) run_steps((int)n);
    stepsSinceSnap_ = n;
}

void Engine::mark_failed(const char* what) noexcept
{
    if (failed_.empty()) failed_ = what ? what : "unknown error";
    unsettled_ = false;
    snap_.valid = false;
    if (stream_) (void)hipStreamSynchronize(stream_);
    (void)hipGetLastError();
    DevStats s;
    if (dStats_ && hipMemcpy(&s, dStats_, sizeof(DevStats), hipMemcpyDeviceToHost) == hipSuccess) hostStep_ = s.step;
    (void)hipGetLastError();
}

void Engine::step(int nsteps)
{
    if (nsteps <= 0) return;
    if (!failed_.empty()) throw std::runtime_error("this handle failed in an earlier call and cannot step on: " + failed_);
    try { step_body(nsteps); }
    catch (const std::exception& e) { mark_failed(e.what()); throw; }
    catch (...) { mark_failed("unknown exception"); throw; }
}

bool Engine::settle_now() const
{
    if (nranks_ > 1 || hasBonded_ || profile_ || (debug_ & DBG_SETTLE_EVERY_CALL)) return true;
    if (!lazyOn_) return false;
    return !lazyMeasured_ || sinceLook_ >= lazyWindow_;
}

void Engine::look(bool callEnd)
{
    look_sync();
    if (!lazyOn_) return;
    if (!adapt_sort_interval())
    {
        replay_from_snapshot();
        if (callEnd)
        {
            kickOwed_ = lazyKick_;
            finish_steps();
            check_launch("step kernels (run again)");
        }
        look_sync();
        if (!adapt_sort_interval()) throw std::runtime_error("lazy re-sort: a skin violation in a run that rebuilds its cells every step");
    }
    if (!callEnd || 2 * sinceLook_ >= lazyWindow_) lazyWindow_ = std::min(window_cap(), 2 * lazyWindow_);
    sinceLook_ = 0;
    if (safeLooks_ > 0) safeLooks_--;
}

void Engine::settle()
{
    if (!unsettled_ || !failed_.empty()) return;
    unsettled_ = false;
    try
    {
        finish_steps();
        check_launch("end-of-call kernels");
        look(true);
        check_overflow();
        prepare_next_call();
        if (lazyOn_)
        {
            choose_optimism();
            if (!rollback_on()) snap_.valid = false;
            else if (!snap_.valid || stepsSinceSnap_ >= kSnapshotKeepSteps) take_snapshot();
        }
    }
    catch (const std::exception& e) { mark_failed(e.what()); throw; }
}

void Engine::step_body(int nsteps)
{
    kickOwed_ = false;
    if (!unsettled_)
    {
        choose_optimism();
        if (rollback_on() && !snap_.valid) take_snapshot();
    }
    int left = nsteps;
    while (left > 0)
    {
        const int n = lazyOn_ ? std::min(left, std::max(1, lazyWindow_ - sinceLook_)) : left;
        run_steps(n);
        left -= n;
        sinceLook_ += n;
        stepsSinceSnap_ += n;
        if (left > 0 && sinceLook_ >= lazyWindow_)
        {
            if (2 * left > lazyWindow_)
            {
                look(false);
                choose_optimism();
                if (rollback_on()) take_snapshot();
            }
            else { run_steps(left); sinceLook_ += left; stepsSinceSnap_ += left; left = 0; }
        }
    }
    kickOwed_ = lazyKick_;
    check_launch("step kernels");
    unsettled_ = true;
    if (settle_now()) settle();
}

int Engine::graph_cycle() const
{
    const int K = lazyOn_ ? lazyK_ : 1;
    return (K == 1) ? 2 : K;
}

bool Engine::can_graph() const
{
    const bool slabGraph = nranks_ > 1 && ownedXch_ && (debug_ & DBG_SLAB_GRAPH) && !(P_.nEq > 0 || P_.tstat == AZTOT_TSTAT_NOSE) && !lazyOn_;
    const bool worthIt = capacity_ <= 2 * kFuseKickMaxAtoms || (debug_ & DBG_GRAPH_ALWAYS);
    return opt_.use_graph && worthIt && (nranks_ == 1 || slabGraph) && !profile_ && !equil_phase();
}

Engine::GraphSlot* Engine::graph_for_state(int cycle)
{
    if (graphCycle_ != cycle) { drop_graphs(); graphCycle_ = cycle; }
    const BufState now = buf_state();
    for (GraphSlot& g : graphs_)
        if (g.before.cur == now.cur && g.before.xyz[0][0] == now.xyz[0][0] && g.before.xyz[1][0] == now.xyz[1][0]) return &g;
    GraphSlot g;
    g.before = now;
    const int sinceBefore = sinceSort_;
    const LaunchNotes notesBefore = notes_;
    const int entryBytesBefore = lists_.entryBytes;
    HIP_CHECK(hipStreamBeginCapture(stream_, hipStreamCaptureModeThreadLocal));
    capturing_ = true;
    try
    {
        sinceSort_ = kNoSort;
        preIntegrated_ = false;
        kickFolded_ = false;
        for (int k = 0; k < cycle; k++) { stepsLeftInRun_ = cycle - 1 - k; launch_step_kernels(); }
    }
    catch (...)
    {
        hipGraph_t broken = nullptr;
        (void)hipStreamEndCapture(stream_, &broken);
        if (broken) (void)hipGraphDestroy(broken);
        capturing_ = false;
        preIntegrated_ = false;
        kickFolded_ = false;
        sinceSort_ = sinceBefore;
        lists_.entryBytes = entryBytesBefore;
        set_buf_state(now);
        adopt_launch_notes(notesBefore);
        throw;
    }
    capturing_ = false;
    HIP_CHECK(hipStreamEndCapture(stream_, &g.graph));
    HIP_CHECK(hipGraphInstantiate(&g.exec, g.graph, nullptr, nullptr, 0));
    g.after = buf_state();
    g.notes = notes_;
    g.entryBytes = lists_.entryBytes;
    lists_.entryBytes = entryBytesBefore;
    set_buf_state(now);
    adopt_launch_notes(notesBefore);
    sinceSort_ = sinceBefore;
    stepsLeftInRun_ = 0;
    graphs_.push_back(g);
    return &graphs_.back();
}

void Engine::run_steps(int nsteps)
{
    int done = 0;
    const bool carryOn = lazyOn_ && (nranks_ == 1 || carryAgreed_) && lists_.on && listsValid_ && lazyK_ > 1 && sinceSort_ < kNoSort / 2 && pair_variant() == 2;
    if (!carryOn) sinceSort_ = kNoSort;
    preIntegrated_ = false;
    while (carryOn && done < nsteps && sinceSort_ < lazyK_ - 1) { stepsLeftInRun_ = nsteps - 1 - done; launch_step_kernels(); done++; }
    const int cycle = graph_cycle();
    if (can_graph() && nsteps - done >= cycle)
    {
        sinceSort_ = kNoSort;
        while (nsteps - done >= cycle)
        {
            GraphSlot* slot = graph_for_state(cycle);
            HIP_CHECK(hipGraphLaunch(slot->exec, stream_));
            done += cycle;
            hostStep_ += cycle;
            rebuilds_ += (lazyOn_ && lazyK_ > 1) ? 1 : cycle;
            set_buf_state(slot->after);
            adopt_launch_notes(slot->notes);
            lists_.entryBytes = slot->entryBytes;
            sinceSort_ = kNoSort;
        }
    }
    preIntegrated_ = false;
    for (; done < nsteps; done++) { stepsLeftInRun_ = nsteps - 1 - done; launch_step_kernels(); }
    stepsLeftInRun_ = 0;
}

void Engine::prepare_next_call()
{
    if (!lazyOn_ || !lazyMeasured_) return;
    if (lists_.on && lazyK_ > 1 && !listsValid_ && sinceSort_ == 0 && pair_variant() == 2)
    {
        P_.cycleStep = 0;
        int32_t rep[LR_COUNT];
        auto record = [&] {
            HIP_CHECK(hipMemsetAsync(&lists_.report[LR_UNLISTED_NOW], 0, sizeof(int32_t), stream_));
            lists_.begin_recording();
            launch_build_lists(pair_launch(P_), PairRange(), lists_.pair_lists());
            check_launch("list building");
            sync();
            HIP_CHECK(hipMemcpy(rep, lists_.report, sizeof(rep), hipMemcpyDeviceToHost));
            unlistedState_ = (rep[LR_UNLISTED_NOW] == 0) ? 1 : 2;
        };
        record();
        bool formatChanged = false;
        if (!(debug_ & DBG_SHORT_LISTS) && lists_.tighten(rep, &formatChanged)) drop_graphs();
        if (formatChanged) record();
        if (nranks_ > 1)
        {
            int32_t h[HI_COUNT];
            post_count_exchange();
            HIP_CHECK(hipStreamSynchronize(stream_));
            HIP_CHECK(hipMemcpy(h, dHaloInfo_, sizeof(h), hipMemcpyDeviceToHost));
            haloInfoPending_ = false;
            adopt_halo_info(h);
        }
        listsValid_ = true;
    }
    if (nranks_ > 1)
    {
        double cannot = (lists_.on && listsValid_ && lazyK_ > 1 && pair_variant() == 2) ? 0.0 : 1.0;
        xch_->allreduce_sum(&cannot, 1, stream_);
        carryAgreed_ = cannot == 0.0;
    }
    if (can_graph()) (void)graph_for_state(graph_cycle());
}

void Engine::look_sync()
{
    if (lazyOn_)
    {
        static_assert(sizeof(Counts) + sizeof(int32_t) * LR_COUNT <= PinnedReadback::kBytes, "the look's block holds Counts and the builder's report");
        hLook_.post(dCounts_, sizeof(Counts), stream_);
        if (lists_.on) hLook_.post(lists_.report, sizeof(int32_t) * LR_COUNT, stream_, sizeof(Counts));
    }
    sync();
}

bool Engine::adapt_sort_interval()
{
    Counts c = *hLook_.as<Counts>();
    bool rebuildNeeded = false;
    const int32_t* rep = hLook_.as<int32_t>(sizeof(Counts));
    if (lists_.on && rep[LR_RECORDED] > 0)
    {
        unlistedAtLook_ = rep[LR_UNLISTED] > 0;
        const ListStore::Verdict v = lists_.adapt(rep, debug_);
        if (v.launchChanged) drop_graphs();
        if (!lists_.on) listsValid_ = false;
        rebuildNeeded = v.rebuild;
    }
    if (nranks_ > 1)
    {
        double v[11] = {0, 0, 0, 0, 0, 0, 0, 0, 0, 0, 0};
        v[10] = rebuildNeeded ? 1.0 : 0.0;
        double mine;
        std::memcpy(&mine, &c.maxStep2, sizeof(mine));
        if (nranks_ <= 8) v[rank_] = mine; else v[0] = 0.0;
        v[8] = c.lazyViolatedEver ? 1.0 : 0.0;
        v[9] = nranks_ > 8 ? mine : 0.0;
        xch_->allreduce_sum(v, 11, stream_);
        rebuildNeeded = v[10] > 0.0;
        double mx = v[9];
        for (int k = 0; k < 8; k++) mx = std::max(mx, v[k]);
        std::memcpy(&c.maxStep2, &mx, sizeof(mx));
        c.lazyViolatedEver = v[8] > 0.0 ? 1 : 0;
        if (c.lazyViolatedEver)
        {
            clear_violation_flag();
            set_interval(1);
            void_measurement();
            lazyMargin_ = std::min(4.0, lazyMargin_ * (4.0 / 3.0));
            if (rebuildNeeded) forget_interval();
            return false;
        }
    }
    HIP_CHECK(hipMemsetAsync(&dCounts_->maxStep2, 0, sizeof(unsigned long long), stream_));
    if (rebuildNeeded) forget_interval();
    lazyMeasured_ = true;
    int K = lazyK_;
    const bool goBack = optimistic_ && (c.lazyViolatedEver != 0 || unlistedAtLook_);
    if (debug_ & DBG_FIXED_INTERVAL)
    {
        if (c.lazyViolatedEver) clear_violation_flag();
        K = lazyCap_;
    }
    else
    {
        const bool violated = c.lazyViolatedEver != 0;
        if (violated)
        {
            clear_violation_flag();
            lazyMargin_ = std::min(4.0, lazyMargin_ * (4.0 / 3.0));
        }
        int fromSpeed = -1;
        if (c.maxStep2 != 0)
        {
            double ms2;
            std::memcpy(&ms2, &c.maxStep2, sizeof(ms2));
            const double len = std::sqrt(ms2);
            const double growth = lastLookLen_ > 0.0 ? (len > 1.1 * lastLookLen_ ? std::min(2.0, len / lastLookLen_) : 1.0) : 1.3 / 1.15;
            lastLookLen_ = len;
            const double raw = len > 0 ? lazySlack_ / ((nranks_ > 1 ? std::max(2.0, lazyMargin_) : lazyMargin_) * growth * len) : 1e9;
            if (std::getenv("AZTOT_VERBOSE"))
                std::fprintf(stderr, "aztot: longest step %.3e A, slack %.3e A, margin %.2f%s: interval up to %.1f steps\n", len, lazySlack_, lazyMargin_, violated ? ", violated" : "", raw);
            static const int allowed[] = {128, 112, 96, 80, 64, 56, 48, 40, 36, 32, 28, 24, 20, 16, 14, 12, 10, 8, 6, 5, 4, 3, 2, 1};
            fromSpeed = 1;
            const int cap = can_graph() ? std::min(lazyCap_, 64) : lazyCap_;
            for (int a : allowed) if (a <= cap && (double)a <= raw) { fromSpeed = a; break; }
            if (!can_graph() && raw >= 1.0) fromSpeed = std::max(fromSpeed, std::min(cap, (int)raw));
        }
        if (violated) K = std::max(1, fromSpeed > 0 ? std::min(K / 2, fromSpeed) : K / 2);
        else if (fromSpeed > 0) K = fromSpeed;
    }
    set_interval(K);
    return !goBack;
}

void Engine::clear_violation_flag()
{
    const int32_t z = 0;
    HIP_CHECK(hipMemcpy(&dCounts_->lazyViolatedEver, &z, sizeof(z), hipMemcpyHostToDevice));
    lazyViolations_++;
}

void Engine::check_overflow()
{
    if (nranks_ <= 1 && !hasBonded_) return;
    Counts c;
    HIP_CHECK(hipMemcpy(&c, dCounts_, sizeof(Counts), hipMemcpyDeviceToHost));
    if (c.overflow) throw std::runtime_error("slab decomposition: a fixed-capacity halo/migration/atom buffer overflowed");
    if (c.bondedMissing)
        throw std::runtime_error("slab decomposition: a bond / angle partner was not resident on the rank that owns the atom "
                                 "(bonded terms must span less than the halo width)");
}

void Engine::get_stats(aztot_stats& out)
{
    const DevStats s = read_stats();
    if (failed_.empty() && s.step != hostStep_) throw std::runtime_error("the host's step count (" + std::to_string(hostStep_) + ") and the device's (" + std::to_string(s.step) + ") differ");
    double v[24];
    v[0] = s.engKin; v[1] = s.engVdW; v[2] = s.engCoul; v[3] = s.engElecField; v[4] = s.engTemp;
    for (int k = 0; k < 6; k++) { v[5 + k] = s.mom[k]; v[11 + k] = (double)s.cross[k]; }
    v[17] = (double)s.dropped; v[18] = s.engBond; v[19] = s.engAngle;
    if (nranks_ > 1) xch_->allreduce_sum(v, 20, stream_);
    std::memset(&out, 0, sizeof(out));
    out.step = s.step;
    out.time = s.step * model_.tSt;
    out.engKin = v[0]; out.engVdW = v[1]; out.engCoul = v[2]; out.engElecField = v[3]; out.engTemp = v[4];
    out.engPot = out.engCoul + out.engVdW;
    out.engBond = v[18]; out.engAngle = v[19];
    out.engCoulRec = s.engCoulRec; out.engCoulConst = s.engCoulConst;
    out.engTot = out.engElecField + out.engVdW + (out.engCoulConst + out.engCoulRec + out.engCoul) + out.engKin + out.engBond +
                 out.engAngle;
    out.temperature = 2.0 * out.engKin * model_.revDegFree * (1.0 / units::kB);
    out.negMom[0] = v[5]; out.posMom[0] = v[6]; out.negMom[1] = v[7]; out.posMom[1] = v[8]; out.negMom[2] = v[9]; out.posMom[2] = v[10];
    out.negCross[0] = (int64_t)v[11]; out.posCross[0] = (int64_t)v[12]; out.negCross[1] = (int64_t)v[13];
    out.posCross[1] = (int64_t)v[14]; out.negCross[2] = (int64_t)v[15]; out.posCross[2] = (int64_t)v[16];
    out.pairs_dropped = (int64_t)v[17];
    out.n_cells = (int64_t)P_.nc[0] * P_.nc[1] * P_.nc[2];
// ... 148 lines not shown
```

aztotmd_amd/csrc/list_store.h:

```cpp
#pragma once
#include "device_resources.h"
#include "model.h"

namespace aztot {

struct StepParams; struct PairLists;

struct ListStore
{
    struct Verdict
    {
        bool rebuild = false;
        bool launchChanged = false;
    };

    bool on = false;
    uint32_t* cand = nullptr;
    int32_t* meta = nullptr;
    uint16_t* pairs = nullptr;
    int32_t* report = nullptr;
    float4* rel = nullptr;
    int candCap = 0, iterCap = 0;
    int candLds = 0, iterLds = 0;
    int stageLds = 0;
    int buildGroups = 0;
    int waves = 1;
    int growths = 0;
    int entryBytes = 2, entryNext = 2;

    void create(const StepParams& P, const Model& m, const aztot_options& opt, int capacity, double listRadius, hipStream_t stream, int rank);
    void regrow(int candCap, int iterCap);
    void release() noexcept;
    PairLists pair_lists() const;
    void lds_for(const int32_t* rep, int& candLds, int& stageLds, int& iterLds, int& buildGroups) const;
    bool tighten(const int32_t* rep, bool* formatChanged = nullptr);
    bool narrow_fits(int maxTile, int candLdsNew, int wavesNew) const;
    void begin_recording() { entryBytes = entryNext; }
    Verdict adapt(const int32_t* rep, unsigned debug);

private:
    void allocate(int candCap, int iterCap);
    int tile_records_for(int maxT) const;
    int stage_records_for(int maxStaged) const;
    int groups_that_fit(int want, int stageLds, int iterLds) const;
    int waves_wanted(double tileRecords, int iters) const;
    DeviceArena mem_;
    const StepParams* P_ = nullptr;
    hipStream_t stream_ = nullptr;
    int capacity_ = 0, rank_ = 0;
    int forcedWaves_ = 0;
    bool wideForGood_ = false;
    size_t ldsMax_ = 0;
};

}
```

aztotmd_amd/csrc/pair_list.hip.h:

```cpp
#pragma once
#include <type_traits>
#include "pair_tile.hip.h"

namespace aztot {

constexpr int kListPreload = 5;
constexpr int kListMinCand = 64 * kListPreload;
__host__ __device__ inline int list_preload(int candLds) { return candLds <= 4 * kWave ? 4 : kListPreload; }
constexpr int kListMinIter = 16;
constexpr int kListMaxSlices = 32;

constexpr int kListMaxWaves = 4;
__host__ __device__ inline int list_atoms_per_wave(int nAtoms, int W) { return (nAtoms + W - 1) >> (W >> 1); }
__host__ __device__ inline int list_slices(int nAtomsOfWave) { const int n = kWave / (nAtomsOfWave > 0 ? nAtomsOfWave : 1); return n > kListMaxSlices ? kListMaxSlices : (n < 1 ? 1 : n); }

inline bool pair_list_tab_mode(const StepParams& P) { return P.potSet == POTSET_ONE_FAMILY && !P.single_lj; }
inline size_t pair_list_lds_bytes(const StepParams& P, const PairLists& L)
{
    const bool tab = pair_list_tab_mode(P);
    const bool generic = !P.single_lj && P.potSet == POTSET_GENERIC;
    const bool radii = !P.single_lj && !tab;
    size_t b = (size_t)(L.candLds + 1) * 24;
    if (tab) b += sizeof(double) * kLjSpecMax * kLjSpecMax * kPairTabStride + (((size_t)L.candLds + 1 + 15) & ~(size_t)15);
    if (radii) b += sizeof(double) * (size_t)(L.candLds + 1);
    if (generic) b += (size_t)(L.candLds + 1 + 7) & ~(size_t)7;
    return b;
}
inline int pair_list_rec_bytes(const StepParams&) { return 24; }
inline int pair_list_entry_scale(const StepParams& P) { return P.single_lj ? 24 : 1; }

__device__ __forceinline__ void fold_drift_atom(const StepParams& P, const SpecTable& S, const NextStep& N, int i, int t, double x, double y, double z,
                                                double xi, double yi, double zi, double vx, double vy, double vz, bool interior, double room2,
                                                double& len2, int& cross, int& violated)
{
    const double x0 = x, y0 = y, z0 = z;
    double dx = 0.0, dy = 0.0, dz = 0.0;
    if (!S.frozen[t]) { dx = vx * P.dt; dy = vy * P.dt; dz = vz * P.dt; x += dx; y += dy; z += dz; }
    len2 = dx * dx + dy * dy + dz * dz;
    bool full = !interior;
    if (interior)
    {
        const double lx = 1.25 * P.csz[0], ly = 1.25 * P.csz[1], lz = 1.25 * P.csz[2];
        const bool far = fabs(xi) > lx || fabs(xi + dx) > lx || fabs(yi) > ly || fabs(yi + dy) > ly || fabs(zi) > lz || fabs(zi + dz) > lz;
        full = __any(far) != 0;
    }
    if (full)
    {
        int c;
        c = image_of(x, P.L[0], P.invL[0]) - image_of(x0, P.L[0], P.invL[0]);
        if (c < 0) cross |= 1; else if (c > 0) cross |= 2;
        c = image_of(y, P.L[1], P.invL[1]) - image_of(y0, P.L[1], P.invL[1]);
        if (c < 0) cross |= 4; else if (c > 0) cross |= 8;
        c = image_of(z, P.L[2], P.invL[2]) - image_of(z0, P.L[2], P.invL[2]);
        if (c < 0) cross |= 16; else if (c > 0) cross |= 32;
    }
    if (!(room2 > 0.0 && len2 < room2))
    {
        const double ex = x - N.R0.x[i], ey = y - N.R0.y[i], ez = z - N.R0.z[i];
        if (ex * ex + ey * ey + ez * ez > P.lazySlack2) violated = 1;
    }
    st_f64(N.xd, i, x); st_f64(N.yd, i, y); st_f64(N.zd, i, z);
}

__device__ __forceinline__ void fold_drift_finish(const StepParams& P, const SpecTable& S, const NextStep& N, int t, double vx, double vy, double vz, double len2,
                                                  int cross, int violated, unsigned long long runBits, unsigned long long maxBits,
                                                  double* __restrict__ partials, int maxBlocks, size_t pb)
{
    const int lane = threadIdx.x & (kWave - 1);
    const unsigned long long mine = (unsigned long long)__double_as_longlong(len2);
    if (__any(mine > maxBits || (P.boundSkip && mine > runBits)))
    {
        double mx = len2;
#pragma unroll
        for (int o = kWave >> 1; o >= 1; o >>= 1) mx = fmax(mx, __shfl_xor(mx, o, kWave));
        if (lane == 0)
        {
            const unsigned long long bits = (unsigned long long)__double_as_longlong(mx);
            if (bits > __hip_atomic_load(&N.cnt->maxStep2, __ATOMIC_RELAXED, __HIP_MEMORY_SCOPE_AGENT)) atomicMax(&N.cnt->maxStep2, bits);
            if (P.boundSkip && bits > __hip_atomic_load(&N.cnt->cycMaxRun, __ATOMIC_RELAXED, __HIP_MEMORY_SCOPE_AGENT)) atomicMax(&N.cnt->cycMaxRun, bits);
        }
    }
    if (__any(violated) && lane == 0)
    {
        if (N.cnt->lazyViolated == 0) N.cnt->lazyViolated = P.cycleStep + 1;
        N.cnt->lazyViolatedEver = 1;
    }
    if (__any(cross != 0))
    {
#pragma unroll
        for (int d = 0; d < 6; d++) if (cross & (1 << d)) atomicAdd(&N.st->specCross[t * 6 + d], 1ULL);
        const double m = S.mass[t];
        next_wall_sum(m * (-vx), cross & 1, 1, 0, partials, maxBlocks, pb); next_wall_sum(m * vx, cross & 2, 2, 1, partials, maxBlocks, pb);
        next_wall_sum(m * (-vy), cross & 4, 4, 2, partials, maxBlocks, pb); next_wall_sum(m * vy, cross & 8, 8, 3, partials, maxBlocks, pb);
        next_wall_sum(m * (-vz), cross & 16, 16, 4, partials, maxBlocks, pb); next_wall_sum(m * vz, cross & 32, 32, 5, partials, maxBlocks, pb);
    }
}

template <int MODE, int VDW, bool ENG, bool MULTI, bool TSTAT = false, int PRE = kListPreload, int EB = 2>
__global__ __launch_bounds__(MULTI ? kWave * kListMaxWaves : kWave) void k_pair_list(StepParams P, SpecTable S, const DevPot* __restrict__ pots, AtomArrays A,
                                                     const int32_t* __restrict__ cellStart, int firstCell, int nCellsRun,
                                                     double* __restrict__ partials, int maxBlocks, const Counts* __restrict__ counts, int blockBase, PairLists L,
                                                     NextStep N)
{
    constexpr bool kOneSpecies = pair_mode_one_species(MODE);
    constexpr bool kRadii = pair_mode_reads_radii(MODE);
    constexpr bool kTab = pair_mode_has_table(MODE);
    constexpr int RECB = 24;
    static_assert(EB == 2 || (EB == 1 && !MULTI && PRE == 4), "one-byte list entries: one wave per cell and the four-group tile only");
    constexpr int ESCALE = (MODE == PM_ONE_LJ && EB == 2) ? 1 : 24;
    constexpr int VPC = 16 / EB;
    constexpr int kTabDoubles = kTab ? kLjSpecMax * kLjSpecMax * kPairTabStride : 0;
    extern __shared__ double ldsList[];
    double* const pairTab = ldsList;
    uint8_t* const ttypT = (uint8_t*)(ldsList + kTabDoubles);
    char* const tb = (char*)(ldsList + kTabDoubles) + (kTab ? ((L.candLds + 1 + 15) & ~15) : 0);
    double* const trad = (double*)(tb + (size_t)(L.candLds + 1) * RECB);
    uint8_t* const ttyp0 = (uint8_t*)(trad + (L.candLds + 1));

    const int lane = threadIdx.x & (kWave - 1), wave = MULTI ? (int)(threadIdx.x >> 6) : 0;
    const int W = MULTI ? L.waves : 1;
    const int per = (nCellsRun + 7) >> 3;
    const int cr = (blockIdx.x & 7) * per + (blockIdx.x >> 3);
    double eV = 0.0, eC = 0.0, dropped = 0.0, eK = 0.0;
    NextAcc nacc;
    if (N.xn) next_acc_clear(nacc);
    const int cell = firstCell + min(cr, nCellsRun - 1);
    const uint32_t* const myList = L.cand + (size_t)cell * L.candCap + lane;
    const uint4* const pl = (const uint4*)(L.pairs + ((size_t)cell * W + wave) * L.iterCap * kWave) + lane;
    constexpr bool kLazyLast = PRE == 4 && !MULTI;
    uint32_t ent[PRE];
#pragma unroll
    for (int u = 0; u < PRE; u++) ent[u] = (kLazyLast && u == PRE - 1) ? 0u : myList[(wave + u * W) * kWave];
    uint4 w = pl[0];
    uint4 w1 = make_uint4(0u, 0u, 0u, 0u);
    if (EB == 2) w1 = pl[kWave];
    const int4 mx = ((const int4*)L.meta)[cell];
    unsigned long long runBits = 0ULL, maxBits = 0ULL;
    if (P.fuseKick == KICK_DRIFT) { runBits = N.cnt->cycMaxRun; maxBits = N.cnt->maxStep2; }
    asm volatile("" ::: "memory");
    const bool violated = P.nranks == 1 && !P.optimistic && slack_violated(P, counts);
    int meta = mx.x;
    if (violated || cr >= nCellsRun || !list_usable(L, meta)) meta = -1;
    if (meta > 0)
    {
        const int T = meta & 0xFFF, nIter = (meta >> 12) & 0xFF;
        const bool lastGroup = !kLazyLast || T > (PRE - 1) * kWave;
        if (kLazyLast)
        {
            if (lastGroup) ent[PRE - 1] = myList[(PRE - 1) * kWave];
            if (EB != 1) asm volatile("" ::: "memory");
        }
        if (EB == 1)
        {
            if (nIter > VPC) w1 = pl[kWave];
            asm volatile("" ::: "memory");
        }
        const int ncy = P.nc[1], ncz = P.nc[2];
        const int lx = mx.y & 1023, cy = (mx.y >> 10) & 1023, cz = (mx.y >> 20) & 1023;
        const int ib = mx.z;
        const double cc0 = (lx + P.cx0) * P.csz[0] + 0.5 * P.csz[0], cc1 = cy * P.csz[1] + 0.5 * P.csz[1], cc2 = cz * P.csz[2] + 0.5 * P.csz[2];
        const DevPot lj = pots[0];
        if (kTab)
        {
            const int np = P.nSpec * P.nSpec;
            if (threadIdx.x < np)
            {
                const DevPot v = pots[lane];
                const int a = lane / P.nSpec, b = lane - a * P.nSpec;
                double* q = pairTab + lane * kPairTabStride;
                q[0] = v.p0; q[1] = v.p1; q[2] = v.p2; q[3] = v.p3; q[4] = v.p4;
                q[5] = v.type ? v.r2cut : -1.0;
                q[6] = (S.charged[a] && S.charged[b]) ? S.charge[a] * S.charge[b] * P.fcoul : 0.0;
                if (v.type == 2) q[3] = 1.0 / v.p1;
                q[7] = (double)v.type;
            }
        }
        const int ncell = mx.w & 0xFFF;
        const int aw = list_atoms_per_wave(ncell, W);
        const int nthis = max(0, min(aw, ncell - wave * aw));
        const int NS = (meta >> 20) & 63;
        const int rcpNS = mx.w >> 12;
        const int slot = (lane * rcpNS) >> 16, slice = lane - slot * NS;
        const bool validI = slot < nthis;
        const int myi = ib + wave * aw + slot;
        const int myl = validI ? myi : ib;
        const double xr = A.x[myl], yr = A.y[myl], zr = A.z[myl];
        double v0x, v0y, v0z, r0x, r0y, r0z;
        if (P.fuseKick || N.xn) { v0x = A.vx[myl]; v0y = A.vy[myl]; v0z = A.vz[myl]; }
        if (N.xn) { r0x = N.R0.x[myl]; r0y = N.R0.y[myl]; r0z = N.R0.z[myl]; }
        double radi = 0.0;
        int ti = 0;
        if (!kOneSpecies) ti = A.type[myl];
        if ((MODE == PM_GENERIC && P.use_radii) || MODE == PM_ONE_SURK) radi = A.rad[myl];
        const int gx0 = lx + P.cx0;
        const bool images = gx0 - P.hw[0] < 0 || gx0 + P.hw[0] >= P.nc[0] || cy - P.hw[1] < 0 || cy + P.hw[1] >= ncy || cz - P.hw[2] < 0 || cz + P.hw[2] >= ncz;
        {
            struct Cand { double x, y, z, rad; int typ; };
            auto fetch = [&](uint32_t e) {
                Cand c;
                const int j = (int)(e & 0x3FFFFFFu);
                c.x = ld_f64(A.x, j); c.y = ld_f64(A.y, j); c.z = ld_f64(A.z, j);
                c.typ = kOneSpecies ? 0 : ld_i32(A.type, j);
                c.rad = ((MODE == PM_GENERIC && P.use_radii) || MODE == PM_ONE_SURK) ? ld_f64(A.rad, j) : 0.0;
                return c;
            };
            auto put = [&](auto IMG, int u, uint32_t e, const Cand& c) {
                if ((MULTI || u >= 4) && u * kWave + lane >= L.candLds) return;
                double xj = c.x, yj = c.y, zj = c.z;
                if (decltype(IMG)::value)
                {
                    xj += (double)((int)((e >> 26) & 3u) - 1) * P.L[0];
                    yj += (double)((int)((e >> 28) & 3u) - 1) * P.L[1];
                    zj += (double)((int)((e >> 30) & 3u) - 1) * P.L[2];
                }
                char* const r = tb + (size_t)(u * kWave + lane + 1) * RECB;
                *(double*)r = xj - cc0; *(double*)(r + 8) = yj - cc1; *(double*)(r + 16) = zj - cc2;
                if (kTab) ttypT[u * kWave + lane + 1] = (uint8_t)c.typ;
                if (kRadii) trad[u * kWave + lane + 1] = c.rad;
                if (MODE == PM_GENERIC) ttyp0[u * kWave + lane + 1] = (uint8_t)c.typ;
            };
            Cand cd[PRE] = {};
#pragma unroll
            for (int u = 0; u < PRE; u++) if (u < PRE - 1 || lastGroup) cd[u] = fetch(ent[u]);
            using ImgYes = std::integral_constant<bool, true>;
            using ImgNo = std::integral_constant<bool, false>;
            if (images)
            {
#pragma unroll
                for (int u = 0; u < PRE; u++) if (u < PRE - 1 || lastGroup) put(ImgYes(), wave + u * W, ent[u], cd[u]);
            }
            else
            {
#pragma unroll
                for (int u = 0; u < PRE; u++) if (u < PRE - 1 || lastGroup) put(ImgNo(), wave + u * W, ent[u], cd[u]);
            }
            if (T > PRE * W * kWave)
            {
                for (int q0 = PRE; (wave + q0 * W) * kWave < T; q0 += 4)
                {
                    uint32_t en[4];
#pragma unroll
                    for (int q = 0; q < 4; q++) en[q] = ((wave + (q0 + q) * W) * kWave < T) ? myList[(wave + (q0 + q) * W) * kWave] : ent[0];
                    const Cand d0 = fetch(en[0]), d1 = fetch(en[1]), d2 = fetch(en[2]), d3 = fetch(en[3]);
                    put(ImgYes(), wave + q0 * W, en[0], d0);
                    if ((wave + (q0 + 1) * W) * kWave < T) put(ImgYes(), wave + (q0 + 1) * W, en[1], d1);
                    if ((wave + (q0 + 2) * W) * kWave < T) put(ImgYes(), wave + (q0 + 2) * W, en[2], d2);
                    if ((wave + (q0 + 3) * W) * kWave < T) put(ImgYes(), wave + (q0 + 3) * W, en[3], d3);
                }
            }
        }
        const double xi = validI ? xr - cc0 : 1e30, yi = validI ? yr - cc1 : 1e30, zi = validI ? zr - cc2 : 1e30;
        constexpr uint32_t dummyOff = 0u;
        if (threadIdx.x == 0)
        {
            char* const r = tb;
            *(double*)r = -1e30; *(double*)(r + 8) = -1e30; *(double*)(r + 16) = -1e30;
            if (kTab) ttypT[0] = 0;
            if (kRadii) trad[0] = 1.0;
            if (MODE == PM_GENERIC) ttyp0[0] = 0;
        }
        __syncthreads();

        PairAcc acc = {0, 0, 0, 0, 0, 0};
        int nDropHalf = 0;
        double ljDropR2 = P.ljDropR2;
        if (kTab) asm volatile("" : "+v"(ljDropR2));
        const PairHot hot = kTab ? pair_hot_in_vgprs(P, lj) : (MODE == PM_ONE_LJ ? pair_hot_lj_in_vgprs(P, lj) : pair_hot(P, lj));
        const int nChunks = (nIter + VPC - 1) / VPC;
        double xj, yj, zj, radj = 0.0;
        int tj = 0;
        auto fetch = [&](uint32_t en, double& x, double& y, double& z, int& ty, double& rd) {
            const uint32_t ko = en * ESCALE;
            x = *(const double*)(tb + ko);
            y = *(const double*)(tb + ko + 8);
            z = *(const double*)(tb + ko + 16);
            if (kTab) ty = ttypT[en];
            if (kRadii) rd = trad[en];
            if (MODE == PM_GENERIC) ty = ttyp0[en];
        };
        fetch(nIter > 0 ? (w.x & (EB == 1 ? 0xFFu : 0xFFFFu)) : dummyOff, xj, yj, zj, tj, radj);
        for (int c = 0; c < nChunks; c++)
        {
            uint4 wn = w1;
            if (c + 2 < nChunks) w1 = pl[(c + 2) * kWave];
            const uint32_t ww[5] = {w.x, w.y, w.z, w.w, wn.x};
#pragma unroll
            for (int u = 0; u < VPC; u++)
            {
                const int t = c * VPC + u;
                if (t >= nIter) break;
                uint32_t kn;
                if (EB == 1) kn = (ww[(u + 1) >> 2] >> (8 * ((u + 1) & 3))) & 0xFFu;
                else kn = ((u + 1) & 1) ? (ww[(u + 1) >> 1] >> 16) : (ww[(u + 1) >> 1] & 0xFFFFu);
                if (u == VPC - 1 && c + 1 >= nChunks) kn = dummyOff;
                double xn, yn, zn, radn = 0.0;
                int tn = 0;
                fetch(kn, xn, yn, zn, tn, radn);
                {
                    const double dx = xi - xj, dy = yi - yj, dz = zi - zj;
                    const double r2 = dx * dx + dy * dy + dz * dz;
                    pair_body<MODE, VDW, true>(P, S, pots, lj, pairTab, true, dx, dy, dz, r2, ti, tj, radi, radj, ljDropR2, nDropHalf, acc, hot);
                }
                xj = xn; yj = yn; zj = zn; tj = tn; radj = radn;
            }
            w = wn;
        }
        if (MODE != PM_GENERIC) acc.dropped += 0.5 * (double)nDropHalf;

        if (NS == 4)
        {
            acc.fx += __shfl_xor(acc.fx, 1, kWave); acc.fy += __shfl_xor(acc.fy, 1, kWave); acc.fz += __shfl_xor(acc.fz, 1, kWave);
            acc.fx += __shfl_xor(acc.fx, 2, kWave); acc.fy += __shfl_xor(acc.fy, 2, kWave); acc.fz += __shfl_xor(acc.fz, 2, kWave);
        }
        else
        {
            int n = NS;
            for (int s = kListMaxSlices / 2; s >= 1; s >>= 1)
            {
                if (s >= n) continue;
                const double ux = __shfl_down(acc.fx, s, kWave), uy = __shfl_down(acc.fy, s, kWave), uz = __shfl_down(acc.fz, s, kWave);
                if (slice < s && slice + s < n) { acc.fx += ux; acc.fy += uy; acc.fz += uz; }
                n = s;
            }
        }
        double dLen2 = 0.0, dvx = 0.0, dvy = 0.0, dvz = 0.0;
        int dCross = 0, dViol = 0;
        if (validI && slice == 0)
        {
            double q = 0.0;
            if (!kOneSpecies) q = S.charge[ti];
            const double fxi = -q * P.E[0] + acc.fx;
            const double fyi = -q * P.E[1] + acc.fy;
            const double fzi = -q * P.E[2] + acc.fz;
            if (P.fuseKick >= KICK_BOTH)
            {
                const double rM = S.rMhdt[ti];
                double vx = v0x + rM * fxi, vy = v0y + rM * fyi, vz = v0z + rM * fzi;
                vx += rM * fxi; vy += rM * fyi; vz += rM * fzi;
                st_f64(A.vx, myi, vx); st_f64(A.vy, myi, vy); st_f64(A.vz, myi, vz);
                if (P.fuseKick == KICK_DRIFT)
                {
                    double room2 = -1.0;
                    if (P.boundSkip)
                    {
                        const float room = __builtin_amdgcn_sqrtf((float)P.lazySlack2) * 0.99999f -
                                           (float)P.cycleStep * (__builtin_amdgcn_sqrtf((float)__longlong_as_double((long long)runBits)) * 1.00001f);
                        if (room > 0.0f) room2 = (double)(room * room);
                    }
                    fold_drift_atom(P, S, N, myi, ti, xr, yr, zr, xi, yi, zi, vx, vy, vz, !images, room2, dLen2, dCross, dViol);
                    dvx = vx; dvy = vy; dvz = vz;
                }
            }
            else
            {
            A.fx[myi] = fxi; A.fy[myi] = fyi; A.fz[myi] = fzi;
            if (P.fuseKick || N.xn)
            {
                const double rM = S.rMhdt[ti], m = S.mass[ti];
                double vx = v0x + rM * fxi, vy = v0y + rM * fyi, vz = v0z + rM * fzi;
                if (ENG && P.fuseKick == KICK_SECOND) eK += (vx * vx + vy * vy + vz * vz) * m;
                if (TSTAT && N.xn)
                    (void)post_tstat_atom(P, S, A, N.st, N.photons, N.uvx, N.uvy, N.uvz, myi, vx, vy, vz, N.st->stepAtSort + (long long)P.cycleStep);
                if (N.xn) next_step_atom(P, S, N, myi, ti, xr, yr, zr, fxi, fyi, fzi, vx, vy, vz, r0x, r0y, r0z, nacc);
                A.vx[myi] = vx; A.vy[myi] = vy; A.vz[myi] = vz;
            }
            }
        }
        if (P.fuseKick == KICK_DRIFT)
            fold_drift_finish(P, S, N, ti, dvx, dvy, dvz, dLen2, dCross, dViol, runBits, maxBits, partials, maxBlocks, (size_t)blockBase + (size_t)blockIdx.x * W + wave);
        if (ENG) { eV = acc.eV; eC = acc.eC; }
        dropped = acc.dropped;
    }
    if (ENG) eV = wave_sum(eV);
    if (ENG && !pair_mode_one_species(MODE)) eC = wave_sum(eC);
    if (__any(dropped != 0.0)) dropped = wave_sum(dropped);
    const size_t pb = (size_t)blockBase + (size_t)blockIdx.x * W + wave;
    if (lane == 0)
    {
        if (ENG)
        {
            partials[(size_t)PS_EVDW * maxBlocks + pb] = eV;
            partials[(size_t)PS_ECOUL * maxBlocks + pb] = eC;
        }
        if (dropped != 0.0) partials[(size_t)PS_DROPPED * maxBlocks + pb] += dropped;
    }
    if (ENG && P.fuseKick == KICK_SECOND)
    {
        eK = wave_sum(eK);
        if (lane == 0) partials[(size_t)PS_EKIN * maxBlocks + pb] = 0.5 * eK;
    }
    if (N.xn)
    {
        next_step_finish(P, N, nacc, partials, maxBlocks, pb);
        if (blockIdx.x == 0 && threadIdx.x == 0) { N.st->step += 1; N.st->pendingKick = 0; }
    }
    else if (N.pendingAfter >= 0 && blockIdx.x == 0 && threadIdx.x == 0) N.st->pendingKick = N.pendingAfter;
    if (P.fuseKick == KICK_DRIFT && threadIdx.x == 0)
    {
        if (blockIdx.x == 0) N.st->step += 1;
        for (int b = blockIdx.x; b < N.driftBlocks; b += gridDim.x) partials[(size_t)PS_EFIELD * maxBlocks + b] = 0.0;
// ... 167 lines not shown
                        {
                            if (keep)
                            {
                                const int pp = T + lanes_below(mask);
                                tile[pp] = make_float4(xf, yf, zf, -(xf * xf + yf * yf + zf * zf));
                                tent[pp] = (uint32_t)(__builtin_amdgcn_readlane(vj, u) + lane) | ((uint32_t)(code & 63) << 26);
                            }
                            T += nk;
                        }
                    }
                }
            }
            __builtin_amdgcn_wave_barrier();
        }
    }
    if (overflow) { no_list(LR_TILE_FULL); return; }
    if ((P.debugMask & DBG_BUILD_PHASE_MASK) == 1) return;

    for (int q = T + lane; q < ((T + 127) & ~127); q += kWave) tile[q] = make_float4(-1e18f, 0.0f, 0.0f, -3e38f);
    for (int q = lane; q < T; q += kWave)
    {
        const uint32_t en = tent[q];
        const int rel = (int)(en & 0x3FFFFFFu) - ib;
        if ((en >> 26) == 0x15u && rel >= 0 && rel < nthis) entJ[rel] = q;
    }
    uint32_t te[kBuildEntRegs];
#pragma unroll
    for (int u = 0; u < kBuildEntRegs; u++) te[u] = (entInRegs && u * kWave < T) ? tent[u * kWave + lane] : 0u;
    __builtin_amdgcn_wave_barrier();
    uint32_t keepAcc = 0u;

    const double h0 = 0.5 * P.csz[0], h1 = 0.5 * P.csz[1], h2 = 0.5 * P.csz[2];
    const double rList = sqrt(P.pruneR2);
    const double ext2 = (h0 + rList) * (h0 + rList) + (h1 + rList) * (h1 + rList) + (h2 + rList) * (h2 + rList);
    const float thrList = (float)(P.pruneR2 + 1.9073486328125e-06 * (4.0 * ext2 + P.pruneR2));
    const int aw = list_atoms_per_wave(nthis, W);
    const int NS = list_slices(aw);
    const int rcpNS = 65536 / NS + 1;
    const int nBlk = (T + 15) >> 4;
    const int nW = (nBlk + 7) >> 3;
    const int c16 = lane & 15, kq = lane >> 4;
    const int permc = (c16 >> 2) + ((c16 & 3) << 2);
    const float* const pa = (const float*)tile + 4 * permc + kq;
    int nIter = 0, hitBase = 0, tooLong = 0;
    auto filter_group = [&](int g0, uint32_t* mb) -> int
    {
        const int a = g0 + c16;
        const bool validA = a < nthis;
        float4 me = make_float4(1e18f, 1e18f, 1e18f, 0.f);
        if (validA) me = L.rel[ib + a];
        const float fB = (kq == 0) ? 2.0f * me.x : (kq == 1) ? 2.0f * me.y : (kq == 2) ? 2.0f * me.z : 1.0f;
        const float cAtom = thrList - (me.x * me.x + me.y * me.y + me.z * me.z);
        const float4_t cw = {cAtom, cAtom, cAtom, cAtom};
        const int kSelf = validA ? entJ[a] : -1;
        int h = 0;
        for (int wd = 0; wd < nW; wd++)
        {
            float av[8];
#pragma unroll
            for (int q = 0; q < 8; q++) av[q] = pa[(8 * wd + q) * 64];
            uint32_t miss = 0u;
#pragma unroll
            for (int q = 0; q < 8; q++)
            {
                const float4_t d = __builtin_amdgcn_mfma_f32_16x16x4f32(av[q], fB, cw, 0, 0, 0);
                miss = __builtin_amdgcn_alignbit(miss, __float_as_uint(d[0]), 31);
                miss = __builtin_amdgcn_alignbit(miss, __float_as_uint(d[1]), 31);
                miss = __builtin_amdgcn_alignbit(miss, __float_as_uint(d[2]), 31);
                miss = __builtin_amdgcn_alignbit(miss, __float_as_uint(d[3]), 31);
            }
            uint32_t m = ~miss;
            if (kSelf >= 0 && (kSelf & 3) == kq && (kSelf >> 7) == wd) m &= ~(0x80000000u >> ((kSelf & 127) >> 2));
            mb[wd * kWave + lane] = m;
            h += __popc(m);
            uint32_t any = m;
            any |= (uint32_t)__builtin_amdgcn_update_dpp(0, (int)any, 0x128, 0xF, 0xF, false);
            any |= (uint32_t)__builtin_amdgcn_update_dpp(0, (int)any, 0x124, 0xF, 0xF, false);
            any |= (uint32_t)__builtin_amdgcn_update_dpp(0, (int)any, 0x122, 0xF, 0xF, false);
            any |= (uint32_t)__builtin_amdgcn_update_dpp(0, (int)any, 0x121, 0xF, 0xF, false);
            if (c16 == wd) keepAcc |= any;
        }
        int below = 0, total = 0, quarters = 0;
#pragma unroll
        for (int q = 0; q < 4; q++)
        {
            const int hq = __shfl(h, c16 | (q << 4), kWave);
            below += (q < kq) ? hq : 0;
            total += hq;
            if (q < 3) quarters |= hq << (10 * q);
        }
        if (!validA) total = 0;
        int incl = total;
#pragma unroll
        for (int o = 1; o < 16; o <<= 1) { const int up = __shfl_up(incl, o, 16); if (c16 >= o) incl += up; }
        const int myOff = hitBase + incl - total;
        hitBase += __shfl(incl, 15, 16);
        if (validA && kq == 0) { entJ[a] = quarters; entN[a] = myOff; entC[a] = total; }
        nIter = max(nIter, ((total + NS - 1) * rcpNS) >> 16);
        if (hitBase > G.hitCap) tooLong = 1;
        return myOff + below;
    };
    auto pop_group = [&](const uint32_t* mb, int at)
    {
        uint16_t* dst = hits + at;
        for (int wd = 0; wd < nW; wd++)
        {
            uint32_t cur = mb[wd * kWave + lane];
            const int base = 128 * wd + kq;
            while (cur != 0u)
            {
                const int p = __clz(cur);
                cur &= ~(0x80000000u >> p);
                *dst++ = (uint16_t)(base + p * 4);
            }
        }
    };
    const bool compact = (P.debugMask & DBG_BUILD_PHASE_MASK) != 2;
    if (beside)
    {
        for (int g0 = 0; g0 < nthis && !tooLong; g0 += 16)
        {
            const int at = filter_group(g0, maskBuf);
            if (!tooLong && compact) pop_group(maskBuf, at);
            __builtin_amdgcn_wave_barrier();
        }
    }
    else
    {
        const int groupWords = G.nWords * kWave;
        uint32_t* mb = maskBuf;
        for (int g0 = 0; g0 < nthis && !tooLong; g0 += 16, mb += groupWords) filter_group(g0, mb);
        __builtin_amdgcn_wave_barrier();
        if (!tooLong && compact)
        {
            mb = maskBuf;
            for (int g0 = 0; g0 < nthis; g0 += 16, mb += groupWords)
            {
                const int a = g0 + c16;
                int at = 0;
                if (a < nthis)
                {
                    const int quarters = entJ[a];
                    at = entN[a] + (kq > 0 ? quarters & 1023 : 0) + (kq > 1 ? (quarters >> 10) & 1023 : 0) + (kq > 2 ? quarters >> 20 : 0);
                }
                pop_group(mb, at);
            }
        }
        __builtin_amdgcn_wave_barrier();
    }
    if ((P.debugMask & DBG_BUILD_PHASE_MASK) >= 2) return;
    nIter = wave_max_int(nIter);
    bool usable = !tooLong && nIter <= ((P.debugMask & DBG_SHORT_LISTS) ? 14 : L.iterCap);
    int kept = 0;
    if (usable)
    {
        __builtin_amdgcn_wave_barrier();
        uint32_t* const myList = L.cand + (size_t)cell * L.candCap;
        auto keep_chunk = [&](int q0, uint32_t entry) {
            const int q = q0 + lane;
            const uint32_t kw = (uint32_t)__shfl((int)keepAcc, ((q & 3) << 4) | (q >> 7), kWave);
            const bool keep = q < T && ((kw << ((q & 127) >> 2)) & 0x80000000u) != 0u;
            const unsigned long long mask = __ballot(keep);
            if (keep)
            {
                const int n = kept + lanes_below(mask);
                remap[q] = (uint16_t)((n + 1) * RECB);
                myList[n] = entry;
            }
            kept += __popcll(mask);
        };
        if (entInRegs)
        {
#pragma unroll
            for (int u = 0; u < kBuildEntRegs; u++) if (u * kWave < T) keep_chunk(u * kWave, te[u]);
        }
        else
            for (int q0 = 0; q0 < T; q0 += kWave) keep_chunk(q0, tent[min(q0 + lane, T - 1)]);
        const int Tpad = max((kept + kWave - 1) & ~(kWave - 1), list_preload(L.candLds) * W * kWave);
        for (int q = kept + lane; q < Tpad; q += kWave) myList[q] = (uint32_t)ib | (0x15u << 26);
        __builtin_amdgcn_wave_barrier();
    }
    const bool narrow = L.entryBytes == 1;
    const bool keptFull = usable && (kept > L.candLds || (narrow && kept > 255));
    if (keptFull) usable = false;
    if (usable)
    {
        const int slot = (lane * rcpNS) >> 16, slice = lane - slot * NS;
        for (int w = 0; w < W; w++)
        {
            const int atom = w * aw + slot;
            int off = 0, cnt = 0;
            if (slot < aw && atom < nthis) { off = entN[atom]; cnt = entC[atom]; }
            const uint16_t* const src = hits + off;
            uint4* const out = (uint4*)(L.pairs + ((size_t)cell * W + w) * L.iterCap * kWave) + lane;
            if (narrow)
            {
                for (int c = 0; c * 16 < nIter; c++)
                {
                    uint32_t v[4] = {0u, 0u, 0u, 0u};
#pragma unroll
                    for (int u = 0; u < 16; u++)
                    {
                        const int e = (c * 16 + u) * NS + slice;
                        const uint32_t r = (e < cnt) ? (uint32_t)remap[src[e]] : 0u;
                        v[u >> 2] |= r << (8 * (u & 3));
                    }
                    out[c * kWave] = make_uint4(v[0], v[1], v[2], v[3]);
                }
                continue;
            }
            for (int c = 0; c * 8 < nIter; c++)
            {
                uint32_t v[8];
#pragma unroll
                for (int u = 0; u < 8; u++)
                {
                    const int e = (c * 8 + u) * NS + slice;
                    v[u] = (e < cnt) ? (uint32_t)remap[src[e]] : 0u;
                }
                out[c * kWave] = make_uint4(v[0] | (v[1] << 16), v[2] | (v[3] << 16), v[4] | (v[5] << 16), v[6] | (v[7] << 16));
            }
        }
    }
    if (lane == 0)
    {
        L.meta[4 * cell] = usable ? (kept | (nIter << 12) | (NS << 20)) : -1;
        L.meta[4 * cell + 2] = ib;
        L.meta[4 * cell + 3] = nthis | (rcpNS << 12);
        if (T > L.noList[LR_MAX_STAGED]) atomicMax(&L.noList[LR_MAX_STAGED], T);
        if (kept > L.noList[LR_MAX_TILE]) atomicMax(&L.noList[LR_MAX_TILE], kept);
        if (usable && nIter > L.noList[LR_MAX_ITERS]) atomicMax(&L.noList[LR_MAX_ITERS], nIter);
        if (nthis > L.noList[LR_MAX_ATOMS]) atomicMax(&L.noList[LR_MAX_ATOMS], nthis);
        if (P.debugMask & DBG_LIST_STATS)
        {
            atomicAdd(&L.noList[LR_SUM_ITERS], nIter); atomicAdd(&L.noList[LR_SUM_CANDS], kept); atomicAdd(&L.noList[LR_SUM_ATOMS], nthis); atomicAdd(&L.noList[LR_SUM_STAGED], T);
            if (nIter > 16) atomicAdd(&L.noList[LR_OVER_16], 1);
        }
        if (!usable) { atomicAdd(&L.noList[LR_UNLISTED], 1); atomicAdd(&L.noList[LR_UNLISTED_NOW], 1); atomicAdd(&L.noList[keptFull ? LR_KEPT_FULL : LR_LIST_FULL], 1); }
    }
}

inline void launch_build_lists(const PairLaunch& C, PairRange R, PairLists L)
{
    pair_range_default(C.P, R);
    if (R.n == 0) return;
    const BuildLds G(L.stageLds, L.iterLds, L.waves, L.buildGroups);
    hipLaunchKernelGGL(k_build_lists, dim3(pair_range_grid(R.n)), dim3(kWave), G.bytes(), C.stream, C.P, C.cellStart, R.first, R.n, L);
}
inline size_t build_lists_lds_bytes(const PairLists& L) { return BuildLds(L.stageLds, L.iterLds, L.waves, L.buildGroups).bytes(); }

template <int MODE, int VDW>
inline void launch_pair_list_as(const PairLaunch& C, PairRange R, PairLists L, NextStep N, bool energies)
{
    const size_t lds = pair_list_lds_bytes(C.P, L);
    const dim3 grid(pair_range_grid(R.n)), block(kWave * L.waves);
    constexpr bool kCanFuseTstat = !pair_mode_reads_radii(MODE);
    const bool four = list_preload(L.candLds) == 4;
    const bool narrow = L.entryBytes == 1;
    if (narrow && (!four || L.waves != 1)) throw std::runtime_error("k_pair_list: one-byte list entries need one wave per cell and a tile of at most 256 records");
#define AZTOT_LAUNCH_LIST_PRE(E, M, T, G, B) hipLaunchKernelGGL((k_pair_list<MODE, VDW, E, M, T, G, B>), grid, block, lds, C.stream, C.P, C.S, C.pots, C.A, C.cellStart, R.first, R.n, C.partials, C.maxBlocks, C.cnt, R.blockBase, L, N)
#define AZTOT_LAUNCH_LIST(E, M, T) do { if (narrow) AZTOT_LAUNCH_LIST_PRE(E, false, T, 4, 1); else if (four) AZTOT_LAUNCH_LIST_PRE(E, M, T, 4, 2); else AZTOT_LAUNCH_LIST_PRE(E, M, T, kListPreload, 2); } while (0)
    if (N.photons)
    {
        if (energies || !kCanFuseTstat) throw std::runtime_error("k_pair_list: the thermostat cannot be fused into this launch");
        if (L.waves == 1) AZTOT_LAUNCH_LIST(false, false, kCanFuseTstat); else AZTOT_LAUNCH_LIST(false, true, kCanFuseTstat);
    }
    else if (L.waves == 1) { if (energies) AZTOT_LAUNCH_LIST(true, false, false); else AZTOT_LAUNCH_LIST(false, false, false); }
    else { if (energies) AZTOT_LAUNCH_LIST(true, true, false); else AZTOT_LAUNCH_LIST(false, true, false); }
#undef AZTOT_LAUNCH_LIST
#undef AZTOT_LAUNCH_LIST_PRE
}

inline int launch_pair_list(const PairLaunch& C, PairRange R, PairLists L, NextStep N = NextStep(), bool energies = true)
{
    pair_range_default(C.P, R);
    if (R.n == 0) return 0;
    AZTOT_PAIR_DISPATCH(C.P, launch_pair_list_as, C, R, L, N, energies);
    return pair_range_grid(R.n) * L.waves;
}

inline int launch_pair_cleanup(const PairLaunch& C, PairRange R, PairLists L, NextStep N = NextStep())
{
    pair_range_default(C.P, R);
    if (R.n == 0) return 0;
    R.blockBase += pair_range_grid(R.n) * L.waves;
    launch_pair_tile(C, R, L, 2, N);
    return pair_cleanup_grid(R.n);
}

}
```

aztotmd_amd/csrc/pair_tile.hip.h:

```cpp
#pragma once
#include "kernels.hip.h"

namespace aztot {

constexpr int kTileCap = 320;
constexpr int kTilePad = 16;
constexpr int kTileLds = kTileCap + kTilePad;
static_assert(kTileLds % 32 == 16, "coordinate arrays must be staggered by half the LDS banks");

typedef float float4_t __attribute__((ext_vector_type(4)));

enum PairMode { PM_GENERIC = 0, PM_ONE_LJ = 1, PM_TAB = 2, PM_TAB_EWALD = 3, PM_ONE_SURK = 4, PM_TAB_FENNELL = 5 };
enum PairVdw { VDW_ANY = 0, VDW_LNJS = 1, VDW_BUCK = 2, VDW_P746 = 3, VDW_BMHS = 4, VDW_MIXED = 5, VDW_LJ_NOCUT = 6, VDW_SURK = 7 };
constexpr bool pair_mode_has_table(int mode) { return mode == PM_TAB || mode == PM_TAB_EWALD || mode == PM_TAB_FENNELL; }
constexpr bool pair_mode_reads_radii(int mode) { return mode == PM_GENERIC || mode == PM_ONE_SURK; }
constexpr bool pair_mode_one_species(int mode) { return mode == PM_ONE_LJ || mode == PM_ONE_SURK; }
constexpr bool pair_mode_ewald(int mode) { return mode == PM_TAB_EWALD; }
constexpr bool pair_mode_fennell(int mode) { return mode == PM_TAB_FENNELL; }
constexpr bool pair_vdw_is_lj(int vdw) { return vdw == VDW_LNJS || vdw == VDW_LJ_NOCUT; }
constexpr bool pair_vdw_no_cut_test(int vdw) { return vdw == VDW_LJ_NOCUT; }
constexpr bool pair_vdw_mixed(int vdw) { return vdw == VDW_MIXED; }


inline bool pair_tile_supported(const StepParams& P)
// ... 155 lines not shown
            const double ar = H.alpha * r;
            const double ex = exp_nonpos<!MASKED>(-ar * ar);
            const double erfcar = erfc_given_exp(ar, ex);
            ra.eC = fma(0.5 * kqq, erfcar * ir - P.el_scale + H.elScale2 * (r - P.rReal), ra.eC);
            f = fma(kqq * ir, (erfcar * r2i + H.daipi2 * ex * ir) - H.elScale2, f);
        }
        else if (pair_mode_ewald(MODE))
        {
            const double kqq = (MASKED || pairOk) ? tabKqq : 0.0;
            const double ar = H.alpha * r;
            const double ex = exp_nonpos<!MASKED>(-ar * ar);
            const double erfcar = erfc_given_exp(ar, ex);
            ra.eC = fma(0.5 * kqq, erfcar * ir, ra.eC);
            f = fma(kqq * ir * r2i, fma(H.daipi2 * r, ex, erfcar), f);
        }
        else if (MODE == PM_TAB && P.elec_type == AZTOT_ELEC_DIRECT)
        {
            const double kqq = (MASKED || pairOk) ? tabKqq : 0.0;
            ra.eC = fma(0.5 * kqq, ir, ra.eC);
            f = fma(kqq * ir, r2i, f);
        }
        double fm = f;
        if (!kLJ || __builtin_expect(__any(r2s < ljDropR2), 0))
        {
            const bool tooBig = f * f > 1e10;
            nDropHalf += tooBig ? 1 : 0;
            fm = tooBig ? 0.0 : f;
        }
        ra.fx = fma(fm, dx, ra.fx); ra.fy = fma(fm, dy, ra.fy); ra.fz = fma(fm, dz, ra.fz);
    }
    else if (live && r2 > 0.0 && r2 <= P.r2Max)
        pair_visit(P, S, pots, dx, dy, dz, r2, ti, tj, radi, radj, ra);
}

template <int LG, int STRIDE, int NW>
__device__ __forceinline__ void tile_filter(const double* tx, const double* ty, const double* tz, const float* tw, int rb, int iters, int slice,
                                            double xi, double yi, double zi, float filtB, double r2Filter, uint32_t (&m)[4])
{
    constexpr int NS = kWave >> LG;
#pragma unroll
    for (int w = 0; w < NW; w++)
    {
        const int tb = rb + w * 32;
        const int nb = min(32, iters - tb);
        uint32_t miss = 0xFFFFFFFFu;
        if (LG == 4)
        {
            const int lane = threadIdx.x & (kWave - 1);
            const int c = lane & 15, k = lane >> 4;
            const int permc = (c >> 2) + ((c & 3) << 2);
            const double* pa = tx + (k == 3 ? 1 : k) * STRIDE + tb * NS + permc;
            const float* pc = tw + tb * NS + k;
            const int nblk = nb >> 2;
#pragma unroll
            for (int q = 0; q < 8; q++)
            {
                if (q < nblk)
                {
                    const float av = (float)pa[q * 16];
                    const float a = (k == 3) ? 1.0f : av;
                    const float4_t cw = {pc[q * 16], pc[q * 16 + 4], pc[q * 16 + 8], pc[q * 16 + 12]};
                    const float4_t d = __builtin_amdgcn_mfma_f32_16x16x4f32(a, filtB, cw, 0, 0, 0);
                    miss = __builtin_amdgcn_alignbit(miss, __float_as_uint(d[0]), 31);
                    miss = __builtin_amdgcn_alignbit(miss, __float_as_uint(d[1]), 31);
                    miss = __builtin_amdgcn_alignbit(miss, __float_as_uint(d[2]), 31);
                    miss = __builtin_amdgcn_alignbit(miss, __float_as_uint(d[3]), 31);
                }
            }
            m[w] = (nb > 0) ? (~miss << (32 - nb)) : 0u;
            continue;
        }
        const double* px = &tx[tb * NS + slice];
        const double* py = &ty[tb * NS + slice];
        const double* pz = &tz[tb * NS + slice];
        for (int b = 0; b < nb; b += 4)
        {
#pragma unroll
            for (int u = 0; u < 4; u++)
            {
                const double dx = xi - px[u * NS], dy = yi - py[u * NS], dz = zi - pz[u * NS];
                const double d = fma(-dz, dz, fma(-dy, dy, fma(-dx, dx, r2Filter)));
                miss = __builtin_amdgcn_alignbit(miss, (uint32_t)(__double_as_longlong(d) >> 32), 31);
            }
            px += 4 * NS; py += 4 * NS; pz += 4 * NS;
        }
        m[w] = (nb > 0) ? (~miss << (32 - nb)) : 0u;
    }
}

template <int MODE, int VDW, int LG, int STRIDE = kTileLds, int NW = 3>
__device__ __forceinline__ void tile_passes(const StepParams& P, const SpecTable& S, const DevPot* __restrict__ pots, const DevPot& lj,
                                            const double* tx, const double* ty, const double* tz, const float* tw, const uint8_t* ttyp, const double* trad,
                                            const double* pairTab, int T, int slice, double xi, double yi, double zi, int ti, double radi,
                                            float filtB, float filtC, PairAcc& acc)
{
    constexpr int NS = kWave >> LG;
    const int iters = ((T + NS - 1) / NS + 3) & ~3;
    const double r2Filter = P.r2Max * (1.0 + 1e-13);
    const double ljDropR2 = P.ljDropR2;
    int nDropHalf = 0;
    if (P.debugMask & DBG_STAGE_ONLY) return;
    for (int rb = 0; rb < iters; rb += 32 * NW)
    {
        uint32_t m[4] = {0u, 0u, 0u, 0u};
        tile_filter<LG, STRIDE, NW>(tx, ty, tz, tw, rb, iters, slice, xi, yi, zi, filtB, r2Filter, m);
        PairAcc& ra = acc;
        uint32_t cur = m[0], nxt = m[1], lst = m[2], ult = m[3];
        int kbase = rb * NS + slice;
        if (__any((cur | nxt | lst | ult) != 0u))
        do
        {
            const bool dry = cur == 0u;
            cur = dry ? nxt : cur;
            nxt = dry ? lst : nxt;
            if (NW > 3) { lst = dry ? ult : lst; ult = dry ? 0u : ult; }
            else lst = dry ? 0u : lst;
            kbase += dry ? 32 * NS : 0;
            constexpr bool kMaskBody = pair_mode_one_species(MODE);
            const bool live = cur != 0u;
            if (kMaskBody ? live : true)
            {
            const int b = __clz(cur | 1u);
            cur &= ~(0x80000000u >> b);
            const int k = (kMaskBody || live) ? kbase + b * NS : T;
            const double dx = xi - tx[k], dy = yi - ty[k], dz = zi - tz[k];
            const double r2 = dx * dx + dy * dy + dz * dz;
            int tj = 0;
            double radj = 0.0;
            if (!pair_mode_one_species(MODE)) tj = ttyp[k];
            if (pair_mode_reads_radii(MODE)) radj = trad[k];
            pair_body<MODE, VDW>(P, S, pots, lj, pairTab, live, dx, dy, dz, r2, ti, tj, radi, radj, ljDropR2, nDropHalf, ra, pair_hot(P, lj));
            }
        } while (__any((cur | nxt | lst | ult) != 0u));
    }

    if (MODE != PM_GENERIC) acc.dropped += 0.5 * (double)nDropHalf;
}

enum ListReport : int
{
    LR_UNLISTED = 0,
    LR_RECORDED = 1,
    LR_UNLISTED_NOW = 2,
    LR_MAX_TILE = 3,
    LR_MAX_ITERS = 4,
    LR_TILE_FULL = 5,
    LR_LIST_FULL = 6,
    LR_KEPT_FULL = 7,
    LR_SUM_ITERS = 8, LR_SUM_CANDS = 9, LR_SUM_ATOMS = 10, LR_SUM_STAGED = 11,
    LR_MAX_STAGED = 12,
    LR_OVER_16 = 13,
    LR_MAX_ATOMS = 14,
    LR_MASK_FULL = 15,
    LR_COUNT = 16,
    LR_NONE = -1
};
struct PairLists
{
    uint32_t* cand = nullptr;
    int32_t* meta = nullptr;
    uint16_t* pairs = nullptr;
    int32_t* noList = nullptr;
    int32_t candCap = 0;
    int32_t iterCap = 0;
    int32_t candLds = 0;
    int32_t stageLds = 0;
    int32_t iterLds = 0;
    int32_t buildGroups = 0;
    int32_t waves = 1;
    int32_t recBytes = 0;
    int32_t entryScale = 0;
    int32_t entryBytes = 2;
    const float4* rel = nullptr;
};
__device__ __forceinline__ bool list_usable(const PairLists& L, int header) { return header >= 0 && (header & 0xFFF) <= L.candLds; }

__device__ __forceinline__ int wave_max_int(int v)
{
#pragma unroll
    for (int o = kWave >> 1; o >= 1; o >>= 1) v = max(v, __shfl_xor(v, o, kWave));
    return v;
}

struct NextStep
{
    double *xn = nullptr, *yn = nullptr, *zn = nullptr;
    RefPos R0{};
    DevStats* st = nullptr;
    Counts* cnt = nullptr;
    const double *photons = nullptr, *uvx = nullptr, *uvy = nullptr, *uvz = nullptr;
    int pendingAfter = -1;
    double *xd = nullptr, *yd = nullptr, *zd = nullptr;
    int driftBlocks = 0;
};

struct NextAcc { double mx, my, mz, stepLen2; int cx, cy, cz, violated; };
__device__ __forceinline__ void next_acc_clear(NextAcc& a) { a.mx = a.my = a.mz = 0.0; a.stepLen2 = 0.0; a.cx = a.cy = a.cz = 0; a.violated = 0; }

__device__ __forceinline__ void next_step_atom(const StepParams& P, const SpecTable& S, const NextStep& N, int i, int t, double x, double y, double z,
                                               double fx, double fy, double fz, double& vx, double& vy, double& vz, double rx, double ry, double rz, NextAcc& a)
{
    const double rM = S.rMhdt[t], m = S.mass[t];
    vx += rM * fx; vy += rM * fy; vz += rM * fz;
    const int ix0 = image_of(x, P.L[0], P.invL[0]), iy0 = image_of(y, P.L[1], P.invL[1]), iz0 = image_of(z, P.L[2], P.invL[2]);
    double dx = 0.0, dy = 0.0, dz = 0.0;
    if (!S.frozen[t]) { dx = vx * P.dt; dy = vy * P.dt; dz = vz * P.dt; x += dx; y += dy; z += dz; }
    a.stepLen2 = dx * dx + dy * dy + dz * dz;
    int c;
    c = image_of(x, P.L[0], P.invL[0]) - ix0;
    if (c < 0) { a.mx = m * (-vx); a.cx = -1; } else if (c > 0) { a.mx = m * vx; a.cx = 1; }
    c = image_of(y, P.L[1], P.invL[1]) - iy0;
    if (c < 0) { a.my = m * (-vy); a.cy = -1; } else if (c > 0) { a.my = m * vy; a.cy = 1; }
    c = image_of(z, P.L[2], P.invL[2]) - iz0;
    if (c < 0) { a.mz = m * (-vz); a.cz = -1; } else if (c > 0) { a.mz = m * vz; a.cz = 1; }
    const double ex = x - rx, ey = y - ry, ez = z - rz;
    if (ex * ex + ey * ey + ez * ez > P.lazySlack2) a.violated = 1;
    if (a.cx) atomicAdd(&N.st->specCross[t * 6 + (a.cx < 0 ? 0 : 1)], 1ULL);
    if (a.cy) atomicAdd(&N.st->specCross[t * 6 + (a.cy < 0 ? 2 : 3)], 1ULL);
    if (a.cz) atomicAdd(&N.st->specCross[t * 6 + (a.cz < 0 ? 4 : 5)], 1ULL);
    N.xn[i] = x; N.yn[i] = y; N.zn[i] = z;
}

__device__ __forceinline__ void next_wall_sum(double m, int c, int want, int slot, double* __restrict__ partials, int maxBlocks, size_t pb)
{
    const double s = wave_sum(c == want ? m : 0.0), b = wave_sum(c == want ? 1.0 : 0.0);
    if ((threadIdx.x & (kWave - 1)) == 0 && b != 0.0) { partials[(size_t)(PS_MOM_XN + slot) * maxBlocks + pb] += s; partials[(size_t)(PS_CNT_XN + slot) * maxBlocks + pb] += b; }
}

__device__ __forceinline__ void next_step_finish(const StepParams& P, const NextStep& N, NextAcc& a, double* __restrict__ partials, int maxBlocks, size_t pb)
{
    const int lane = threadIdx.x & (kWave - 1);
    double mx = a.stepLen2;
#pragma unroll
    for (int o = kWave >> 1; o >= 1; o >>= 1) mx = fmax(mx, __shfl_xor(mx, o, kWave));
    if (lane == 0)
    {
        const unsigned long long bits = (unsigned long long)__double_as_longlong(mx);
        if (bits > __hip_atomic_load(&N.cnt->maxStep2, __ATOMIC_RELAXED, __HIP_MEMORY_SCOPE_AGENT)) atomicMax(&N.cnt->maxStep2, bits);
    }
    if (__any(a.violated) && lane == 0)
    {
        if (N.cnt->lazyViolated == 0) N.cnt->lazyViolated = P.cycleStep + 1;
        N.cnt->lazyViolatedEver = 1;
    }
    if (__any((a.cx | a.cy | a.cz) != 0))
    {
        next_wall_sum(a.mx, a.cx, -1, 0, partials, maxBlocks, pb); next_wall_sum(a.mx, a.cx, 1, 1, partials, maxBlocks, pb);
        next_wall_sum(a.my, a.cy, -1, 2, partials, maxBlocks, pb); next_wall_sum(a.my, a.cy, 1, 3, partials, maxBlocks, pb);
        next_wall_sum(a.mz, a.cz, -1, 4, partials, maxBlocks, pb); next_wall_sum(a.mz, a.cz, 1, 5, partials, maxBlocks, pb);
    }
}

template <int MODE, int VDW, bool CLEANUP>
__global__ __launch_bounds__(kWave, pair_mode_has_table(MODE) ? 3 : 1) void k_pair_tile(StepParams P, SpecTable S, const DevPot* __restrict__ pots, AtomArrays A,
                                                     const int32_t* __restrict__ cellStart, int firstCell, int nCellsRun,
                                                     double* __restrict__ partials, int maxBlocks, const Counts* __restrict__ counts, int blockBase,
                                                     PairLists L, NextStep N, SplitArgs Z)
{
    constexpr bool onlyUnlisted = CLEANUP;
    const bool widened = P.lazySlack2 > 0.0 && P.nranks == 1 && slack_violated(P, counts);
    if (widened)
    {
        for (int k = 0; k < 3; k++) { P.hw[k] += 1; P.nOff[k] = 2 * P.hw[k] + 1; }
        P.pruneR2 = 1e300;
    }
    constexpr bool kOneSpecies = pair_mode_one_species(MODE);
    __shared__ double txyz[3 * kTileLds];
    __shared__ float tw[kTileLds];
    double* const tx = txyz;
    double* const ty = txyz + kTileLds;
    double* const tz = txyz + 2 * kTileLds;
    __shared__ uint8_t ttyp[!kOneSpecies ? kTileLds : 1];
    __shared__ double trad[pair_mode_reads_radii(MODE) ? kTileLds : 1];
    __shared__ double pairTab[pair_mode_has_table(MODE) ? kLjSpecMax * kLjSpecMax * kPairTabStride : 1];
    __shared__ int32_t entJ[kWave], entN[kWave], entC[kWave];

    const int lane = threadIdx.x;
    PairAcc acc = {0, 0, 0, 0, 0, 0};
    double eV = 0.0, eC = 0.0, dropped = 0.0, eK = 0.0;
    NextAcc nacc;
    next_acc_clear(nacc);
    const DevPot lj = pots[0];
    if (pair_mode_has_table(MODE))
    {
        const int np = P.nSpec * P.nSpec;
        if (lane < np)
        {
            const DevPot v = pots[lane];
            const int a = lane / P.nSpec, b = lane - a * P.nSpec;
            double* q = pairTab + lane * kPairTabStride;
            q[0] = v.p0; q[1] = v.p1; q[2] = v.p2; q[3] = v.p3; q[4] = v.p4;
            q[5] = v.type ? v.r2cut : -1.0;
            q[6] = (S.charged[a] && S.charged[b]) ? S.charge[a] * S.charge[b] * P.fcoul : 0.0;
            if (v.type == 2) q[3] = 1.0 / v.p1;
            q[7] = (double)v.type;
        }
        __builtin_amdgcn_wave_barrier();
    }
    const int per = (nCellsRun + 7) >> 3;
    const int rowStep = (int)(gridDim.x >> 3);
    bool cleanupIdle = false;
    if (onlyUnlisted && !widened) cleanupIdle = L.noList[LR_UNLISTED_NOW] == 0;
    const int nSplit = CLEANUP ? 1 : Z.n;
    const int sub = (int)(blockIdx.x >> 3) & (nSplit - 1);
    for (int rowBase = (int)(blockIdx.x >> 3) / nSplit; rowBase < per && !cleanupIdle; rowBase += CLEANUP ? kWave * rowStep : per)
    {
    unsigned long long todo = 1ULL;
    if (CLEANUP)
    {
        const int myRow = rowBase + lane * rowStep;
        const int myCr = (blockIdx.x & 7) * per + myRow;
        bool need = myRow < per && myCr < nCellsRun;
        if (!widened && need) need = !list_usable(L, L.meta[4 * (firstCell + myCr)]);
        todo = __ballot(need);
    }
    else if ((blockIdx.x & 7) * per + rowBase >= nCellsRun) todo = 0ULL;
    while (todo != 0ULL)
    {
        const int rowK = CLEANUP ? __ffsll((long long)todo) - 1 : 0;
        todo &= todo - 1ULL;
        const int cr = (blockIdx.x & 7) * per + rowBase + rowK * rowStep;
        const int cell = firstCell + cr;
        const int ncy = P.nc[1], ncz = P.nc[2];
        const int cz = cell % ncz, cy = (cell / ncz) % ncy, lx = cell / (ncy * ncz);
        const int ib = cellStart[cell], ie = cellStart[cell + 1];
// ... 332 lines not shown
```

Baseline: 945.7 ns/day.

## Store pair-list candidates as 16-bit offsets from per-group bases with separate image bytes

Adds a narrow candidate format for cells whose list uses one-byte entries. The builder writes a 32-bit base per wave group, a 16-bit offset per candidate, and a separate image-code byte used only by boundary cells. The pair kernel reads about half the candidate bytes per cell and reconstructs atom indices with wraparound clamping. Cells whose candidates span more than 65535 indices fall back to unlisted, which also permanently switches the store back to the wide format. This adds template variants, graph-slot bookkeeping and an extra rebuild path.

```diff
diff --git a/aztotmd_amd/api.py b/aztotmd_amd/api.py
--- a/aztotmd_amd/api.py
+++ b/aztotmd_amd/api.py
@@ -145,6 +145,7 @@
     DBG_NO_FUSE_NEXT = 131072
     DBG_FUSE_NEXT = 262144
     DBG_CHECK_EVERY_ATOM = 524288
+    DBG_WIDE_CANDIDATES = 1048576
     DBG_LIST_STATS = 2097152
     DBG_KICK_POST_SPLIT = 4194304
     DBG_GRAPH_ALWAYS = 8388608
diff --git a/aztotmd_amd/csrc/device_md.h b/aztotmd_amd/csrc/device_md.h
--- a/aztotmd_amd/csrc/device_md.h
+++ b/aztotmd_amd/csrc/device_md.h
@@ -101,6 +101,7 @@
     DBG_NO_FUSE_NEXT = 131072,
     DBG_FUSE_NEXT = 262144,
     DBG_CHECK_EVERY_ATOM = 524288,
+    DBG_WIDE_CANDIDATES = 1048576,
     DBG_LIST_STATS = 2097152,
     DBG_KICK_POST_SPLIT = 4194304,
     DBG_GRAPH_ALWAYS = 8388608,
diff --git a/aztotmd_amd/csrc/engine.h b/aztotmd_amd/csrc/engine.h
--- a/aztotmd_amd/csrc/engine.h
+++ b/aztotmd_amd/csrc/engine.h
@@ -189,7 +189,7 @@
         bool ekinFromPair = false;
         bool lastStepEquil = false;
     } notes_;
-    struct GraphSlot { BufState before, after; LaunchNotes notes; hipGraph_t graph = nullptr; hipGraphExec_t exec = nullptr; int entryBytes = 2; };
+    struct GraphSlot { BufState before, after; LaunchNotes notes; hipGraph_t graph = nullptr; hipGraphExec_t exec = nullptr; int entryBytes = 2, candBytes = 4; };
     void adopt_launch_notes(const LaunchNotes& n) { const int ever = std::max(notes_.blocksEver, n.blocksEver); notes_ = n; notes_.blocksEver = ever; }
     std::vector<GraphSlot> graphs_;
     int graphCycle_ = 0;
diff --git a/aztotmd_amd/csrc/engine.hip b/aztotmd_amd/csrc/engine.hip
--- a/aztotmd_amd/csrc/engine.hip
+++ b/aztotmd_amd/csrc/engine.hip
@@ -479,7 +479,7 @@
 
 void ListStore::create(const StepParams& P, const Model& m, const aztot_options& opt, int capacity, double listRadius, hipStream_t stream, int rank)
 {
-    P_ = &P; stream_ = stream; capacity_ = capacity; rank_ = rank;
+    P_ = &P; stream_ = stream; capacity_ = capacity; rank_ = rank; nAtoms_ = m.nAt;
     forcedWaves_ = (opt.waves_per_cell == 1 || opt.waves_per_cell == 2 || opt.waves_per_cell == 4) ? opt.waves_per_cell : 0;
     if (P.ncxLocal > 1023 || P.nc[1] > 1023 || P.nc[2] > 1023) throw std::runtime_error("more than 1023 cells along an axis");
     int devLds = 0;
@@ -496,6 +496,7 @@
     iters = std::max(2 * kListMinIter, (iters + 7) & ~7);
     if (const char* e = std::getenv("AZTOT_CAND_CAP")) cand = std::atoi(e);
     if (const char* e = std::getenv("AZTOT_ITER_CAP")) iters = std::atoi(e);
+    if (const char* e = std::getenv("AZTOT_CAND_SPAN")) candSpan = std::max(0, std::min(65535, std::atoi(e)));
     try { allocate(cand, iters); }
     catch (const std::exception&)
     {
@@ -528,6 +529,7 @@
     candLds = stageLds = candCapNew; iterLds = iterCapNew;
     buildGroups = groups_that_fit(4 * waves, stageLds, iterLds);
     entryBytes = entryNext = 2;
+    candBytes = candNext = 4;
     {
         std::vector<int32_t> mx(4 * nc, 0);
         const int ncy = P.nc[1], ncz = P.nc[2];
@@ -573,6 +575,7 @@
         pl.candCap = candCap; pl.iterCap = iterCap; pl.candLds = candLds; pl.stageLds = stageLds; pl.iterLds = iterLds; pl.recBytes = pair_list_rec_bytes(*P_); pl.waves = waves;
         pl.buildGroups = buildGroups;
         pl.entryBytes = entryBytes; pl.entryScale = entryBytes == 1 ? 1 : pair_list_entry_scale(*P_);
+        pl.candBytes = candBytes; pl.candSpan = candSpan; pl.lastAtom = capacity_ - 1; pl.candWrap = nAtoms_;
         pl.rel = rel;
     }
     return pl;
@@ -634,6 +637,22 @@
     return P_->nranks == 1 && !(P_->debugMask & DBG_WIDE_ENTRIES) && !wideForGood_ && wavesNew == 1 && list_preload(candLdsNew) == 4 && maxTile <= 255;
 }
 
+void ListStore::choose_cand_format()
+{
+    candNext = (entryNext == 1 && !(P_->debugMask & DBG_WIDE_CANDIDATES) && !candWideForGood_ && !pair_list_generic_mode(*P_)) ? 2 : 4;
+}
+
+bool ListStore::span_seen_on_the_spot(const int32_t* rep)
+{
+    if (candBytes != 2 || rep[LR_CAND_SPAN] <= 0) return false;
+    candWideForGood_ = true;
+    choose_cand_format();
+    const int32_t unlisted = std::max(0, rep[LR_UNLISTED] - rep[LR_CAND_SPAN]), zero = 0;
+    HIP_CHECK(hipMemcpy(&report[LR_UNLISTED], &unlisted, sizeof(int32_t), hipMemcpyHostToDevice));
+    HIP_CHECK(hipMemcpy(&report[LR_CAND_SPAN], &zero, sizeof(int32_t), hipMemcpyHostToDevice));
+    return true;
+}
+
 bool ListStore::tighten(const int32_t* rep, bool* formatChanged)
 {
     if (formatChanged) *formatChanged = false;
@@ -644,6 +663,7 @@
     if (entryNext == 2 && narrow_fits(rep[LR_MAX_TILE], std::min(candLds, c), waves))
     {
         entryNext = 1;
+        choose_cand_format();
         lds_for(rep, c, s, i, g);
         changed = true;
         if (formatChanged) *formatChanged = true;
@@ -671,7 +691,9 @@
     HIP_CHECK(hipMemsetAsync(&report[LR_UNLISTED], 0, sizeof(int32_t) * 2, stream_));
     HIP_CHECK(hipMemsetAsync(&report[LR_TILE_FULL], 0, sizeof(int32_t) * 3, stream_));
     HIP_CHECK(hipMemsetAsync(&report[LR_MASK_FULL], 0, sizeof(int32_t), stream_));
+    HIP_CHECK(hipMemsetAsync(&report[LR_CAND_SPAN], 0, sizeof(int32_t), stream_));
     const int tileFull = rep[LR_TILE_FULL], keptFull = rep[LR_KEPT_FULL], listFull = rep[LR_LIST_FULL], maskFull = rep[LR_MASK_FULL], recorded = rep[LR_RECORDED], unlisted = rep[LR_UNLISTED];
+    const int spanFull = rep[LR_CAND_SPAN];
     if (std::getenv("AZTOT_VERBOSE"))
         std::fprintf(stderr, "aztot: lists recorded since the last look: %d cells, %d of them without a list (%d: staging full, %d: tile full, %d: list full, %d: mask buffer full); most staged %d of %d (LDS %d), largest tile %d (LDS %d), longest list %d of %d (LDS %d), most atoms %d (LDS %d groups, builder %zu B)\n",
                      recorded, unlisted, tileFull, keptFull, listFull, maskFull, rep[LR_MAX_STAGED], candCap, stageLds, rep[LR_MAX_TILE], candLds, rep[LR_MAX_ITERS], iterCap, iterLds, rep[LR_MAX_ATOMS], buildGroups,
@@ -696,6 +718,8 @@
         v.launchChanged = true;
         lds_for(rep, candLdsNew, stageLdsNew, iterLdsNew, groupsNew);
     }
+    if (spanFull > 0 && !candWideForGood_) { candWideForGood_ = true; v.rebuild = v.launchChanged = true; }
+    choose_cand_format();
     if (wWant > waves && !forcedWaves_ && !frozen)
     {
         const int itersNew = std::max(2 * kListMinIter, ((int)(rep[LR_MAX_ITERS] * (double)waves / wWant * 1.3) + 8 + 7) & ~7);
@@ -718,7 +742,7 @@
         candLds = candLdsNew; stageLds = stageLdsNew; iterLds = iterLdsNew; buildGroups = groupsNew;
         v.launchChanged = true;
     }
-    if (on && (double)unlisted > 0.02 * (double)recorded && !frozen && tileFull + keptFull + listFull + maskFull < unlisted / 2)
+    if (on && (double)unlisted > 0.02 * (double)recorded && !frozen && tileFull + keptFull + listFull + maskFull + spanFull < unlisted / 2)
     {
         on = false;
         v.launchChanged = true;
@@ -998,6 +1022,7 @@
                 }
                 const PairLaunch CL = pair_launch(QL);
                 if (profile_ && !capturing_ && pl.entryBytes == 1) timers_.count("narrow_lists");
+                if (profile_ && !capturing_ && pl.candBytes == 2) timers_.count("narrow_cands");
                 timed("pair_list", [&] { splitBlocks = launch_pair_list(CL, PairRange(), pl, nx, wantEnergies); });
                 if (!skipCleanup)
                     timed("pair_cleanup", [&] { splitBlocks += launch_pair_cleanup(C, PairRange(), pl, nx); });
@@ -1472,6 +1497,7 @@
     const int sinceBefore = sinceSort_;
     const LaunchNotes notesBefore = notes_;
     const int entryBytesBefore = lists_.entryBytes;
+    const int candBytesBefore = lists_.candBytes;
     HIP_CHECK(hipStreamBeginCapture(stream_, hipStreamCaptureModeThreadLocal));
     capturing_ = true;
     try
@@ -1491,6 +1517,7 @@
         kickFolded_ = false;
         sinceSort_ = sinceBefore;
         lists_.entryBytes = entryBytesBefore;
+        lists_.candBytes = candBytesBefore;
         set_buf_state(now);
         adopt_launch_notes(notesBefore);
         throw;
@@ -1501,7 +1528,9 @@
     g.after = buf_state();
     g.notes = notes_;
     g.entryBytes = lists_.entryBytes;
+    g.candBytes = lists_.candBytes;
     lists_.entryBytes = entryBytesBefore;
+    lists_.candBytes = candBytesBefore;
     set_buf_state(now);
     adopt_launch_notes(notesBefore);
     sinceSort_ = sinceBefore;
@@ -1531,6 +1560,7 @@
             set_buf_state(slot->after);
             adopt_launch_notes(slot->notes);
             lists_.entryBytes = slot->entryBytes;
+            lists_.candBytes = slot->candBytes;
             sinceSort_ = kNoSort;
         }
     }
@@ -1559,6 +1589,7 @@
         bool formatChanged = false;
         if (!(debug_ & DBG_SHORT_LISTS) && lists_.tighten(rep, &formatChanged)) drop_graphs();
         if (formatChanged) record();
+        if (formatChanged && lists_.span_seen_on_the_spot(rep)) { drop_graphs(); record(); }
         if (nranks_ > 1)
         {
             int32_t h[HI_COUNT];
diff --git a/aztotmd_amd/csrc/list_store.h b/aztotmd_amd/csrc/list_store.h
--- a/aztotmd_amd/csrc/list_store.h
+++ b/aztotmd_amd/csrc/list_store.h
@@ -27,6 +27,8 @@
     int waves = 1;
     int growths = 0;
     int entryBytes = 2, entryNext = 2;
+    int candBytes = 4, candNext = 4;
+    int candSpan = 65535;
 
     void create(const StepParams& P, const Model& m, const aztot_options& opt, int capacity, double listRadius, hipStream_t stream, int rank);
     void regrow(int candCap, int iterCap);
@@ -35,7 +37,8 @@
     void lds_for(const int32_t* rep, int& candLds, int& stageLds, int& iterLds, int& buildGroups) const;
     bool tighten(const int32_t* rep, bool* formatChanged = nullptr);
     bool narrow_fits(int maxTile, int candLdsNew, int wavesNew) const;
-    void begin_recording() { entryBytes = entryNext; }
+    bool span_seen_on_the_spot(const int32_t* rep);
+    void begin_recording() { entryBytes = entryNext; candBytes = candNext; }
     Verdict adapt(const int32_t* rep, unsigned debug);
 
 private:
@@ -48,7 +51,10 @@
     const StepParams* P_ = nullptr;
     hipStream_t stream_ = nullptr;
     int capacity_ = 0, rank_ = 0;
+    int nAtoms_ = 0;
     int forcedWaves_ = 0;
+    void choose_cand_format();
+    bool candWideForGood_ = false;
     bool wideForGood_ = false;
     size_t ldsMax_ = 0;
 };
diff --git a/aztotmd_amd/csrc/pair_list.hip.h b/aztotmd_amd/csrc/pair_list.hip.h
--- a/aztotmd_amd/csrc/pair_list.hip.h
+++ b/aztotmd_amd/csrc/pair_list.hip.h
@@ -10,11 +10,20 @@
 constexpr int kListMinIter = 16;
 constexpr int kListMaxSlices = 32;
 
+constexpr int kNarrowCandGroups = 4;
+constexpr int kNarrowCandEntOff = 4 * kNarrowCandGroups;
+constexpr int kNarrowCandImgOff = kNarrowCandEntOff + 2 * kWave * kNarrowCandGroups;
+static_assert(kNarrowCandImgOff + kWave * kNarrowCandGroups <= 4 * kListMinCand, "the narrow candidate format fits the smallest slot");
+
 constexpr int kListMaxWaves = 4;
 __host__ __device__ inline int list_atoms_per_wave(int nAtoms, int W) { return (nAtoms + W - 1) >> (W >> 1); }
 __host__ __device__ inline int list_slices(int nAtomsOfWave) { const int n = kWave / (nAtomsOfWave > 0 ? nAtomsOfWave : 1); return n > kListMaxSlices ? kListMaxSlices : (n < 1 ? 1 : n); }
 
 inline bool pair_list_tab_mode(const StepParams& P) { return P.potSet == POTSET_ONE_FAMILY && !P.single_lj; }
+inline bool pair_list_generic_mode(const StepParams& P)
+{
+    return !P.single_lj && P.potSet != POTSET_ONE_SURK && !(P.potSet == POTSET_ONE_FAMILY && P.vdwFamily >= VDW_LNJS && P.vdwFamily <= VDW_LJ_NOCUT);
+}
 inline size_t pair_list_lds_bytes(const StepParams& P, const PairLists& L)
 {
     const bool tab = pair_list_tab_mode(P);
@@ -96,7 +105,7 @@
     }
 }
 
-template <int MODE, int VDW, bool ENG, bool MULTI, bool TSTAT = false, int PRE = kListPreload, int EB = 2>
+template <int MODE, int VDW, bool ENG, bool MULTI, bool TSTAT = false, int PRE = kListPreload, int EB = 2, int CB = 4>
 __global__ __launch_bounds__(MULTI ? kWave * kListMaxWaves : kWave) void k_pair_list(StepParams P, SpecTable S, const DevPot* __restrict__ pots, AtomArrays A,
                                                      const int32_t* __restrict__ cellStart, int firstCell, int nCellsRun,
                                                      double* __restrict__ partials, int maxBlocks, const Counts* __restrict__ counts, int blockBase, PairLists L,
@@ -107,6 +116,7 @@
     constexpr bool kTab = pair_mode_has_table(MODE);
     constexpr int RECB = 24;
     static_assert(EB == 2 || (EB == 1 && !MULTI && PRE == 4), "one-byte list entries: one wave per cell and the four-group tile only");
+    static_assert(CB == 4 || (CB == 2 && EB == 1 && PRE == kNarrowCandGroups), "narrow candidate entries: the kernel of the one-byte list entries only");
     constexpr int ESCALE = (MODE == PM_ONE_LJ && EB == 2) ? 1 : 24;
     constexpr int VPC = 16 / EB;
     constexpr int kTabDoubles = kTab ? kLjSpecMax * kLjSpecMax * kPairTabStride : 0;
@@ -128,13 +138,20 @@
     const uint32_t* const myList = L.cand + (size_t)cell * L.candCap + lane;
     const uint4* const pl = (const uint4*)(L.pairs + ((size_t)cell * W + wave) * L.iterCap * kWave) + lane;
     constexpr bool kLazyLast = PRE == 4 && !MULTI;
+    const uint16_t* const myList16 = (const uint16_t*)((const char*)(L.cand + (size_t)cell * L.candCap) + kNarrowCandEntOff) + lane;
     uint32_t ent[PRE];
 #pragma unroll
-    for (int u = 0; u < PRE; u++) ent[u] = (kLazyLast && u == PRE - 1) ? 0u : myList[(wave + u * W) * kWave];
+    for (int u = 0; u < PRE; u++)
+    {
+        if (CB == 2) ent[u] = (u == PRE - 1) ? 0u : (uint32_t)myList16[u * kWave];
+        else ent[u] = (kLazyLast && u == PRE - 1) ? 0u : myList[(wave + u * W) * kWave];
+    }
     uint4 w = pl[0];
     uint4 w1 = make_uint4(0u, 0u, 0u, 0u);
     if (EB == 2) w1 = pl[kWave];
     const int4 mx = ((const int4*)L.meta)[cell];
+    uint4 cb = make_uint4(0u, 0u, 0u, 0u);
+    if (CB == 2) cb = *(const uint4*)(L.cand + (size_t)cell * L.candCap);
     unsigned long long runBits = 0ULL, maxBits = 0ULL;
     if (P.fuseKick == KICK_DRIFT) { runBits = N.cnt->cycMaxRun; maxBits = N.cnt->maxStep2; }
     asm volatile("" ::: "memory");
@@ -147,7 +164,7 @@
         const bool lastGroup = !kLazyLast || T > (PRE - 1) * kWave;
         if (kLazyLast)
         {
-            if (lastGroup) ent[PRE - 1] = myList[(PRE - 1) * kWave];
+            if (lastGroup) ent[PRE - 1] = CB == 2 ? (uint32_t)myList16[(PRE - 1) * kWave] : myList[(PRE - 1) * kWave];
             if (EB != 1) asm volatile("" ::: "memory");
         }
         if (EB == 1)
@@ -196,22 +213,38 @@
         const bool images = gx0 - P.hw[0] < 0 || gx0 + P.hw[0] >= P.nc[0] || cy - P.hw[1] < 0 || cy + P.hw[1] >= ncy || cz - P.hw[2] < 0 || cz + P.hw[2] >= ncz;
         {
             struct Cand { double x, y, z, rad; int typ; };
-            auto fetch = [&](uint32_t e) {
+            const uint32_t cbase[4] = {cb.x, cb.y, cb.z, cb.w};
+            auto index_of = [&](int u, uint32_t e) -> int {
+                if (CB == 2)
+                {
+                    const uint32_t j = cbase[u & 3] + e;
+                    return (int)min(min(j, j - (uint32_t)L.candWrap), (uint32_t)L.lastAtom);
+                }
+                return (int)(e & 0x3FFFFFFu);
+            };
+            uint32_t img[PRE] = {};
+            if (CB == 2 && images)
+            {
+                const uint8_t* const myImg = (const uint8_t*)(L.cand + (size_t)cell * L.candCap) + kNarrowCandImgOff + lane;
+#pragma unroll
+                for (int u = 0; u < PRE; u++) if (u < PRE - 1 || lastGroup) img[u] = myImg[u * kWave];
+            }
+            auto code_of = [&](int u, uint32_t e) -> uint32_t { return CB == 2 ? img[u < PRE ? u : 0] : (e >> 26); };
+            auto fetch = [&](int j) {
                 Cand c;
-                const int j = (int)(e & 0x3FFFFFFu);
                 c.x = ld_f64(A.x, j); c.y = ld_f64(A.y, j); c.z = ld_f64(A.z, j);
                 c.typ = kOneSpecies ? 0 : ld_i32(A.type, j);
                 c.rad = ((MODE == PM_GENERIC && P.use_radii) || MODE == PM_ONE_SURK) ? ld_f64(A.rad, j) : 0.0;
                 return c;
             };
-            auto put = [&](auto IMG, int u, uint32_t e, const Cand& c) {
+            auto put = [&](auto IMG, int u, uint32_t code, const Cand& c) {
                 if ((MULTI || u >= 4) && u * kWave + lane >= L.candLds) return;
                 double xj = c.x, yj = c.y, zj = c.z;
                 if (decltype(IMG)::value)
                 {
-                    xj += (double)((int)((e >> 26) & 3u) - 1) * P.L[0];
-                    yj += (double)((int)((e >> 28) & 3u) - 1) * P.L[1];
-                    zj += (double)((int)((e >> 30) & 3u) - 1) * P.L[2];
+                    xj += (double)((int)(code & 3u) - 1) * P.L[0];
+                    yj += (double)((int)((code >> 2) & 3u) - 1) * P.L[1];
+                    zj += (double)((int)((code >> 4) & 3u) - 1) * P.L[2];
                 }
                 char* const r = tb + (size_t)(u * kWave + lane + 1) * RECB;
                 *(double*)r = xj - cc0; *(double*)(r + 8) = yj - cc1; *(double*)(r + 16) = zj - cc2;
@@ -221,31 +254,31 @@
             };
             Cand cd[PRE] = {};
 #pragma unroll
-            for (int u = 0; u < PRE; u++) if (u < PRE - 1 || lastGroup) cd[u] = fetch(ent[u]);
+            for (int u = 0; u < PRE; u++) if (u < PRE - 1 || lastGroup) cd[u] = fetch(index_of(u, ent[u]));
             using ImgYes = std::integral_constant<bool, true>;
             using ImgNo = std::integral_constant<bool, false>;
             if (images)
             {
 #pragma unroll
-                for (int u = 0; u < PRE; u++) if (u < PRE - 1 || lastGroup) put(ImgYes(), wave + u * W, ent[u], cd[u]);
+                for (int u = 0; u < PRE; u++) if (u < PRE - 1 || lastGroup) put(ImgYes(), wave + u * W, code_of(u, ent[u]), cd[u]);
             }
             else
             {
 #pragma unroll
-                for (int u = 0; u < PRE; u++) if (u < PRE - 1 || lastGroup) put(ImgNo(), wave + u * W, ent[u], cd[u]);
-            }
-            if (T > PRE * W * kWave)
+                for (int u = 0; u < PRE; u++) if (u < PRE - 1 || lastGroup) put(ImgNo(), wave + u * W, 0x15u, cd[u]);
+            }
+            if (CB == 4 && T > PRE * W * kWave)
             {
                 for (int q0 = PRE; (wave + q0 * W) * kWave < T; q0 += 4)
                 {
                     uint32_t en[4];
 #pragma unroll
                     for (int q = 0; q < 4; q++) en[q] = ((wave + (q0 + q) * W) * kWave < T) ? myList[(wave + (q0 + q) * W) * kWave] : ent[0];
-                    const Cand d0 = fetch(en[0]), d1 = fetch(en[1]), d2 = fetch(en[2]), d3 = fetch(en[3]);
-                    put(ImgYes(), wave + q0 * W, en[0], d0);
-                    if ((wave + (q0 + 1) * W) * kWave < T) put(ImgYes(), wave + (q0 + 1) * W, en[1], d1);
-                    if ((wave + (q0 + 2) * W) * kWave < T) put(ImgYes(), wave + (q0 + 2) * W, en[2], d2);
-                    if ((wave + (q0 + 3) * W) * kWave < T) put(ImgYes(), wave + (q0 + 3) * W, en[3], d3);
+                    const Cand d0 = fetch((int)(en[0] & 0x3FFFFFFu)), d1 = fetch((int)(en[1] & 0x3FFFFFFu)), d2 = fetch((int)(en[2] & 0x3FFFFFFu)), d3 = fetch((int)(en[3] & 0x3FFFFFFu));
+                    put(ImgYes(), wave + q0 * W, en[0] >> 26, d0);
+                    if ((wave + (q0 + 1) * W) * kWave < T) put(ImgYes(), wave + (q0 + 1) * W, en[1] >> 26, d1);
+                    if ((wave + (q0 + 2) * W) * kWave < T) put(ImgYes(), wave + (q0 + 2) * W, en[2] >> 26, d2);
+                    if ((wave + (q0 + 3) * W) * kWave < T) put(ImgYes(), wave + (q0 + 3) * W, en[3] >> 26, d3);
                 }
             }
         }
@@ -719,6 +752,9 @@
     nIter = wave_max_int(nIter);
     bool usable = !tooLong && nIter <= ((P.debugMask & DBG_SHORT_LISTS) ? 14 : L.iterCap);
     int kept = 0;
+    const bool candNarrow = L.candBytes == 2;
+    uint32_t* const keptEnt = beside ? (uint32_t*)(lds + G.remap_bytes()) : tent;
+    bool spanFull = false;
     if (usable)
     {
         __builtin_amdgcn_wave_barrier();
@@ -732,7 +768,8 @@
             {
                 const int n = kept + lanes_below(mask);
                 remap[q] = (uint16_t)((n + 1) * RECB);
-                myList[n] = entry;
+                if (!candNarrow) myList[n] = entry;
+                else if (n < kNarrowCandGroups * kWave) keptEnt[n] = entry;
             }
             kept += __popcll(mask);
         };
@@ -744,12 +781,42 @@
         else
             for (int q0 = 0; q0 < T; q0 += kWave) keep_chunk(q0, tent[min(q0 + lane, T - 1)]);
         const int Tpad = max((kept + kWave - 1) & ~(kWave - 1), list_preload(L.candLds) * W * kWave);
-        for (int q = kept + lane; q < Tpad; q += kWave) myList[q] = (uint32_t)ib | (0x15u << 26);
+        if (!candNarrow)
+            for (int q = kept + lane; q < Tpad; q += kWave) myList[q] = (uint32_t)ib | (0x15u << 26);
+        else if (kept < kNarrowCandGroups * kWave)
+        {
+            __builtin_amdgcn_wave_barrier();
+            const int gx0 = lx + P.cx0;
+            const bool images = gx0 - P.hw[0] < 0 || gx0 + P.hw[0] >= P.nc[0] || cy - P.hw[1] < 0 || cy + P.hw[1] >= ncy || cz - P.hw[2] < 0 || cz + P.hw[2] >= ncz;
+            uint16_t* const out16 = (uint16_t*)((char*)myList + kNarrowCandEntOff);
+            uint8_t* const out8 = (uint8_t*)myList + kNarrowCandImgOff;
+            uint32_t myBase = 0u;
+#pragma unroll
+            for (int u = 0; u < kNarrowCandGroups; u++)
+            {
+                const int n = u * kWave + lane;
+                const uint32_t e = n < kept ? keptEnt[n] : ((uint32_t)ib | (0x15u << 26));
+                int j = (int)(e & 0x3FFFFFFu);
+                int lo = -wave_max_int(-j), hi = wave_max_int(j);
+                if (hi - lo > L.candSpan)
+                {
+                    if (j < (L.candWrap >> 1)) j += L.candWrap;
+                    lo = -wave_max_int(-j); hi = wave_max_int(j);
+                    if (hi - lo > L.candSpan || lo >= L.candWrap) spanFull = true;
+                }
+                out16[n] = (uint16_t)(j - lo);
+                if (images) out8[n] = (uint8_t)(e >> 26);
+                if (lane == u) myBase = (uint32_t)lo;
+            }
+            if (lane < kNarrowCandGroups) myList[lane] = myBase;
+        }
         __builtin_amdgcn_wave_barrier();
     }
     const bool narrow = L.entryBytes == 1;
     const bool keptFull = usable && (kept > L.candLds || (narrow && kept > 255));
     if (keptFull) usable = false;
+    spanFull = spanFull && usable;
+    if (spanFull) usable = false;
     if (usable)
     {
         const int slot = (lane * rcpNS) >> 16, slice = lane - slot * NS;
@@ -803,7 +870,7 @@
             atomicAdd(&L.noList[LR_SUM_ITERS], nIter); atomicAdd(&L.noList[LR_SUM_CANDS], kept); atomicAdd(&L.noList[LR_SUM_ATOMS], nthis); atomicAdd(&L.noList[LR_SUM_STAGED], T);
             if (nIter > 16) atomicAdd(&L.noList[LR_OVER_16], 1);
         }
-        if (!usable) { atomicAdd(&L.noList[LR_UNLISTED], 1); atomicAdd(&L.noList[LR_UNLISTED_NOW], 1); atomicAdd(&L.noList[keptFull ? LR_KEPT_FULL : LR_LIST_FULL], 1); }
+        if (!usable) { atomicAdd(&L.noList[LR_UNLISTED], 1); atomicAdd(&L.noList[LR_UNLISTED_NOW], 1); atomicAdd(&L.noList[spanFull ? LR_CAND_SPAN : keptFull ? LR_KEPT_FULL : LR_LIST_FULL], 1); }
     }
 }
 
@@ -825,8 +892,10 @@
     const bool four = list_preload(L.candLds) == 4;
     const bool narrow = L.entryBytes == 1;
     if (narrow && (!four || L.waves != 1)) throw std::runtime_error("k_pair_list: one-byte list entries need one wave per cell and a tile of at most 256 records");
-#define AZTOT_LAUNCH_LIST_PRE(E, M, T, G, B) hipLaunchKernelGGL((k_pair_list<MODE, VDW, E, M, T, G, B>), grid, block, lds, C.stream, C.P, C.S, C.pots, C.A, C.cellStart, R.first, R.n, C.partials, C.maxBlocks, C.cnt, R.blockBase, L, N)
-#define AZTOT_LAUNCH_LIST(E, M, T) do { if (narrow) AZTOT_LAUNCH_LIST_PRE(E, false, T, 4, 1); else if (four) AZTOT_LAUNCH_LIST_PRE(E, M, T, 4, 2); else AZTOT_LAUNCH_LIST_PRE(E, M, T, kListPreload, 2); } while (0)
+    const bool narrowCand = L.candBytes == 2;
+    if (narrowCand && (!narrow || MODE == PM_GENERIC)) throw std::runtime_error("k_pair_list: narrow candidate entries need one-byte list entries and a specialised pair mode");
+#define AZTOT_LAUNCH_LIST_PRE(E, M, T, G, B, CBY) hipLaunchKernelGGL((k_pair_list<MODE, VDW, E, M, T, G, B, CBY>), grid, block, lds, C.stream, C.P, C.S, C.pots, C.A, C.cellStart, R.first, R.n, C.partials, C.maxBlocks, C.cnt, R.blockBase, L, N)
+#define AZTOT_LAUNCH_LIST(E, M, T) do { if (narrowCand) { if constexpr (MODE != PM_GENERIC) AZTOT_LAUNCH_LIST_PRE(E, false, T, 4, 1, 2); } else if (narrow) AZTOT_LAUNCH_LIST_PRE(E, false, T, 4, 1, 4); else if (four) AZTOT_LAUNCH_LIST_PRE(E, M, T, 4, 2, 4); else AZTOT_LAUNCH_LIST_PRE(E, M, T, kListPreload, 2, 4); } while (0)
     if (N.photons)
     {
         if (energies || !kCanFuseTstat) throw std::runtime_error("k_pair_list: the thermostat cannot be fused into this launch");
diff --git a/aztotmd_amd/csrc/pair_tile.hip.h b/aztotmd_amd/csrc/pair_tile.hip.h
--- a/aztotmd_amd/csrc/pair_tile.hip.h
+++ b/aztotmd_amd/csrc/pair_tile.hip.h
@@ -331,7 +331,8 @@
     LR_OVER_16 = 13,
     LR_MAX_ATOMS = 14,
     LR_MASK_FULL = 15,
-    LR_COUNT = 16,
+    LR_CAND_SPAN = 16,
+    LR_COUNT = 17,
     LR_NONE = -1
 };
 struct PairLists
@@ -350,6 +351,10 @@
     int32_t recBytes = 0;
     int32_t entryScale = 0;
     int32_t entryBytes = 2;
+    int32_t candBytes = 4;
+    int32_t lastAtom = 0;
+    int32_t candWrap = 0;
+    int32_t candSpan = 65535;
     const float4* rel = nullptr;
 };
 __device__ __forceinline__ bool list_usable(const PairLists& L, int header) { return header >= 0 && (header & 0xFFF) <= L.candLds; }
```

Result: no change. 939.2 ns/day (-0.7%).
